# aws/sagemaker-xgboost-container

Hardware: NVIDIA H100
Metric: boosting rounds/sec (higher is better)
Workload: dtype int64

## Files before the change

### sagemaker-xgboost-container_b200/csrc/grow.cu

```cuda
#include "grow.h"
#include <algorithm>
#include <cmath>
#include <cstdlib>
#include <cstring>
#include "comm.h"

namespace b200 {

__global__ void pack_tree_kernel(TreeArrays t, const int* n_nodes, DevNode* out, int cap) {
  const int nn = *n_nodes;
  for (int i = blockIdx.x * blockDim.x + threadIdx.x; i < cap; i += gridDim.x * blockDim.x) {
    DevNode d;
    if (i < nn) { d.cond = t.split_cond[i]; d.left = t.left[i]; d.right = t.right[i]; d.fidx_dl = (unsigned)t.split_index[i] | ((unsigned)t.default_left[i] << 31); }
    else { d.cond = 0.f; d.left = -1; d.right = -1; d.fidx_dl = 0; }
    out[i] = d;
  }
}
__global__ void snapshot_h_kernel(const GH64* slot, long long* cache, size_t entries) {
  for (size_t e = (size_t)blockIdx.x * blockDim.x + threadIdx.x; e < entries; e += (size_t)gridDim.x * blockDim.x) cache[e] = slot[e].h;
}
__global__ void slot_from_cache_kernel(GH64* slot, const long long* cache, size_t entries) {
  for (size_t e = (size_t)blockIdx.x * blockDim.x + threadIdx.x; e < entries; e += (size_t)gridDim.x * blockDim.x) { GH64 v; v.g = 0; v.h = cache[e]; slot[e] = v; }
}
__global__ void gather_u32_kernel(const unsigned* src, const unsigned* idx, unsigned* dst, int64_t n) {
  const int64_t i = (int64_t)blockIdx.x * blockDim.x + threadIdx.x;
  if (i < n) dst[i] = src[idx[i]];
}

void* PinnedPool::take(size_t bytes) {
  bytes = (bytes + 255) & ~(size_t)255;
  while (cur < chunks.size() && off + bytes > chunks[cur].second) { ++cur; off = 0; }
  if (cur >= chunks.size()) { size_t sz = std::max<size_t>(bytes, 4u << 20); char* p = nullptr; CUDA_OK(cudaMallocHost(&p, sz)); chunks.emplace_back(p, sz); off = 0; }
  void* r = chunks[cur].first + off; off += bytes; return r;
}
static bool tail_by_position(const BinnedMatrix& bm) { return bm.tw == 4 && !bm.tail_in_gather; }

size_t TreeBuilder::carve(GrowState& gs, uintptr_t base) const {
  const size_t N = cap_nodes, L = max_level_nodes, nblocks = ngroups + (tw > 0 ? 1 : 0);
  size_t off = 0;
  auto take = [&](auto*& p, size_t bytes) { p = reinterpret_cast<std::remove_reference_t<decltype(p)>>(base + off); off += (bytes + 255) & ~(size_t)255; };
  take(gs.seg_begin, 4 * N); take(gs.seg_count, 4 * N); take(gs.hist_slot, 4 * N); take(gs.node_sum, 16 * N); take(gs.root_gain, 4 * N); take(gs.weight, 4 * N);
  take(gs.best, sizeof(SplitCand) * N); take(gs.best_group, sizeof(SplitCand) * N * nblocks);
  take(gs.level_nodes, 4 * (size_t)(kMaxDepth + 1) * L); take(gs.level_count, 4 * (kMaxDepth + 2));
  take(gs.build_nid, 4 * L); take(gs.build_sub_nid, 4 * L); take(gs.build_parent_slot, 4 * L); take(gs.build_count, 4); take(gs.build_prefix, 4 * (L + 1));
  take(gs.part_action, 4 * L); take(gs.tile_prefix, 4 * (L + 1));
  take(gs.tile_desc, 8 * ((size_t)max_tiles + 1)); gs.part_ctl = (unsigned*)(gs.tile_desc + max_tiles);
  take(gs.n_leaves, 4); take(gs.scales, 16); take(gs.absmax, 8);
  take(gs.depth, 4 * N); take(gs.open, N); take(gs.n_slots, 4); take(gs.lg_done, 4); take(gs.lower, 4 * N); take(gs.upper, 4 * N);
  return off;
}

void TreeBuilder::ensure(const BinnedMatrix& bm, int max_depth_, int K, int lg_iters_, int n_ic_) {
  const bool tail_pos_ = tail_by_position(bm);
  const int64_t stride_ = (bm.n + 63) & ~(int64_t)63;
  if (n == bm.n && F == bm.F && ngroups == bm.ngroups && tw == bm.tw && tail_pos == tail_pos_ && max_depth == max_depth_ && lg_iters == lg_iters_ &&
      n_ic == n_ic_ && gpair.n >= (size_t)stride_ * K + 512) return;
  if (lg_iters_ == 0) B200_CHECK(max_depth_ >= 1 && max_depth_ <= kMaxDepth, "max_depth must be in [1, 16] for the B200 depth-wise hist builder");
  n = bm.n; F = bm.F; ngroups = bm.ngroups; tw = bm.tw; tail_pos = tail_pos_; max_depth = max_depth_; lg_iters = lg_iters_; n_ic = n_ic_;
  gp_stride = stride_; root_h_valid = false;
  cudaStream_t s = engine_stream();
  if (peer_reduce_active()) {
    peer_reduce_close();
    DevBuf<unsigned> bar; bar.alloc(1); bar.zero(s);
    Comm::get().allreduce_max_u32(bar.p, 1, s);
    Comm::get().sync_stream(s);
  }
  for (auto& tg : graphs) tg.destroy();
  size_t pool_slots; int max_nodes;
  if (lg_iters > 0) {
    max_nodes = 2 * lg_iters + 1; max_level_nodes = 2; region = 0;
    pool_slots = (size_t)lg_iters + kLgFirstFreeSlot;
  } else {
    max_nodes = (1 << (max_depth + 1)) - 1; max_level_nodes = 1 << (max_depth - 1); region = max_level_nodes;
    pool_slots = 2 * (size_t)region;
  }
  cap_nodes = (max_nodes + 15) & ~15;
  slot_stride = hist_slot_entries(ngroups, tw);
  const size_t pool_bytes = pool_slots * slot_stride * sizeof(GH64);
  size_t free_b = 0, total_b = 0; cudaMemGetInfo(&free_b, &total_b);
  B200_CHECK(pool_bytes < free_b / 2 + hist_pool.n * sizeof(GH64), "histogram pool for this max_depth / max_leaves / feature count does not fit in device memory");
  hist_pool.alloc(pool_slots * slot_stride);
  gpair.alloc((size_t)gp_stride * K + 512); gpair.zero(s); err.alloc(1); tree_index_dev.alloc(1);
  if (!leaf_scale.p) { leaf_scale.alloc(1); set_leaf_scale(1.0f); }
  root_h_cache.alloc(slot_stride);
  const bool routed = routes(lg_iters, max_depth);
  for (int i = 0; i < 2; ++i) { const size_t m = i == 0 || !routed ? (size_t)n : 0; ridx[i].alloc(m); gp[i].alloc(m); tl[i].alloc(tail_pos ? m : 0); }
  route_tiles = routed ? (unsigned)((n + kRouteTile - 1) / kRouteTile) : 0u;
  node_of_row.alloc(routed ? (size_t)n : 0);
  route_counts.alloc(routed && max_depth >= 2 ? ((size_t)1 << (max_depth - 2)) * route_tiles : 0);
  max_tiles = (unsigned)((n + kPartTile - 1) / kPartTile) + max_level_nodes + 1;
  scratch.alloc(3 * (size_t)max_level_nodes + 8);
  state_block.alloc(carve(gs, 0)); state_block.zero(s);
  carve(gs, (uintptr_t)state_block.p);
  tree_block.alloc(tree_block_bytes(cap_nodes));
  const TreeBlock tb = tree_block_layout(tree_block.p, cap_nodes);
  gs.n_nodes = tb.n_nodes; ta = tb.t; packed.alloc(cap_nodes);
  ic_path.alloc(n_ic ? (size_t)cap_nodes * F : 0); ic_allowed.alloc(n_ic ? (size_t)cap_nodes * F : 0);
  ic_sets.alloc((size_t)n_ic * F); ic_sets_host.clear();
  hist_configure();
  global_n = n;
  if (Comm::get().distributed()) {
    peer_reduce_setup({{hist_pool.p, hist_pool.n * sizeof(GH64)}, {state_block.p, state_block.n}}, s);
    DevBuf<double> dsum; dsum.alloc(1); double v = (double)n;
    CUDA_OK(cudaMemcpyAsync(dsum.p, &v, sizeof v, cudaMemcpyHostToDevice, s));
    Comm::get().allreduce_sum_f64(dsum.p, 1, s);
    CUDA_OK(cudaMemcpyAsync(&v, dsum.p, sizeof v, cudaMemcpyDeviceToHost, s));
    Comm::get().sync_stream(s);
    global_n = (int64_t)v;
  }
}

float* TreeBuilder::ensure_adaptive() {
  if (adapt.ensure(n, max_leaves(), cap_nodes)) for (auto& tg : graphs) tg.destroy();
  return adapt.resid.p;
}

void TreeBuilder::set_leaf_scale(float v) {
  cudaStream_t s = engine_stream();
  CUDA_OK(cudaMemcpyAsync(leaf_scale.p, &v, sizeof v, cudaMemcpyHostToDevice, s));
  Comm::get().sync_stream(s);
}

const unsigned char* TreeBuilder::upload_mask(const std::string& mask, int tree_index) {
  cudaStream_t s = engine_stream(); feat_mask.ensure(mask.size());
  CUDA_OK(cudaMemcpyAsync(feat_mask.p, mask.data(), mask.size(), cudaMemcpyHostToDevice, s));
  CUDA_OK(cudaMemcpyAsync(tree_index_dev.p, &tree_index, sizeof(int), cudaMemcpyHostToDevice, s));
  Comm::get().sync_stream(s); return feat_mask.p;
}
template <typename T> static T* upload_changed(DevBuf<T>& d, std::vector<T>& host, const std::vector<T>& v) {
  if (v == host && d.n >= v.size()) return d.p;
  cudaStream_t s = engine_stream(); d.ensure(v.size());
  CUDA_OK(cudaMemcpyAsync(d.p, v.data(), sizeof(T) * v.size(), cudaMemcpyHostToDevice, s));
  Comm::get().sync_stream(s); host = v; return d.p;
}

const int* TreeBuilder::upload_monotone(const std::vector<int>& mono, int F_) {
  if (mono.empty()) return nullptr;
  B200_CHECK((int)mono.size() <= F_, "monotone_constraints has more entries than the data has features");
  std::vector<int> mh(mono); mh.resize((size_t)F_, 0);
  return upload_changed(monotone_dev, monotone_host, mh);
}
void TreeBuilder::upload_interaction(const std::vector<std::vector<int>>& ic, int F_) {
  if (ic.empty()) return;
  std::vector<unsigned char> sets(ic.size() * (size_t)F_, 0);
  for (size_t si = 0; si < ic.size(); ++si)
    for (int f : ic[si]) { B200_CHECK(f < F_, "interaction_constraints names feature " + std::to_string(f) + " but the data has " + std::to_string(F_) + " features"); sets[si * F_ + f] = 1; }
  upload_changed(ic_sets, ic_sets_host, sets);
}
HistArgs TreeBuilder::hist_args(const BinnedMatrix& bm, int k) const {
  HistArgs ha{}; ha.bins = bm.bins; ha.bins_tail = bm.bins_tail; ha.n = bm.n; ha.row_stride = bm.ngroups * kSlots; ha.tw = bm.tw;
  ha.bins_gather = bm.bins_gather; ha.gather_stride = bm.gather_stride;
  ha.tail_in_gather = bm.tail_in_gather;
  ha.gpair = gpair.p + (size_t)k * gp_stride;
  ha.build_count = gs.build_count; ha.build_nid = gs.build_nid; ha.build_prefix = gs.build_prefix; ha.seg_begin = gs.seg_begin;
  ha.hist_slot = gs.hist_slot; ha.scales = gs.scales; ha.hist_pool = hist_pool.p; ha.node_sum = gs.node_sum; ha.ngroups = bm.ngroups;
  ha.accumulate_sum = 1; ha.window_rows = window_rows_for(global_n);
  return ha;
}

EvalArgs TreeBuilder::eval_args(const TreeInputs& in, int level, const unsigned char* feat_mask) const {
  const BinnedMatrix& bm = in.bm;
  EvalArgs ea{}; ea.hist_pool = hist_pool.p; ea.gs = gs; ea.cut_ptrs = in.cut_ptrs; ea.feat_mask = feat_mask; ea.p = in.p; ea.F = bm.F;
  ea.ngroups = bm.ngroups; ea.tw = bm.tw; ea.ntail = bm.ntail; ea.has_missing = bm.has_missing; ea.level = level; ea.max_level_nodes = max_level_nodes;
  ea.colsample_bynode = in.mask ? in.colsample_bynode : 1.0f; ea.seed = in.seed; ea.tree_index = tree_index_dev.p; ea.monotone = in.monotone;
  ea.node_allowed = in.n_ic > 0 ? ic_allowed.p : nullptr;
  return ea;
}
ApplyArgs TreeBuilder::apply_args(const TreeInputs& in, int level, int next_base, int next_half) const {
  const BinnedMatrix& bm = in.bm;
  ApplyArgs aa{}; aa.gs = gs; aa.tree = ta; aa.cut_ptrs = in.cut_ptrs; aa.cut_vals = in.cut_vals; aa.min_vals = in.min_vals;
  aa.p = in.p; aa.scratch = scratch.p; aa.nblocks = bm.ngroups + (bm.tw > 0 ? 1 : 0); aa.level = level; aa.max_level_nodes = max_level_nodes;
  aa.next_base = next_base; aa.next_half = next_half; aa.monotone = in.monotone;
  if (in.n_ic > 0) { aa.node_path = ic_path.p; aa.node_allowed = ic_allowed.p; aa.ic_sets = ic_sets.p; aa.n_ic_sets = in.n_ic; aa.F = bm.F; }
  return aa;
}
template <class Launch> void TreeBuilder::timed(ProfKind kind, Launch launch) {
  if (!profile) { launch(); return; }
  ProfEvent e; e.kind = kind; e.launches = g_kernel_launches;
  CUDA_OK(cudaEventCreate(&e.a)); CUDA_OK(cudaEventCreate(&e.b));
  CUDA_OK(cudaEventRecord(e.a, engine_stream()));
  launch();
  e.launches = g_kernel_launches - e.launches;
  CUDA_OK(cudaEventRecord(e.b, engine_stream()));
  prof_events.push_back(e);
}

constexpr int kRootRows = -1;
void TreeBuilder::enqueue(const TreeInputs& in) {
  cudaStream_t s = engine_stream();
  const BinnedMatrix& bm = in.bm;
  const int k = in.k, D = in.p.max_depth;
  const bool dist = in.world > 1;
  const int num_sms = engine_num_sms();
  launch_init_tree(gs, ta, (unsigned)bm.n, s);
  if (in.root_mode == 2) { slot_from_cache_kernel<<<num_sms, 256, 0, s>>>(hist_pool.p, root_h_cache.p, slot_stride); ++g_kernel_launches; CUDA_OK(cudaGetLastError()); }
  else CUDA_OK(cudaMemsetAsync(hist_pool.p, 0, slot_stride * sizeof(GH64), s));
  const bool g_only = in.root_mode != 0;
  const int pay = g_only ? 4 : 8;
  const bool carry_tail = tail_by_position(bm);
  const bool routed = routes(in.lg_iters, D);
  if (profile && routed) {
    prof_part_row_bytes[0] = 3;
    prof_part_row_bytes[1] = 4;
    prof_part_row_bytes[2] = pay + 4 + pay + (carry_tail ? 8 : 0);
  } else if (profile) {
    prof_part_row_bytes[0] = pay + (carry_tail ? 4 : 0) + 1;
    prof_part_row_bytes[2] = 4 + pay + (carry_tail ? 4 : 0);
    prof_part_row_bytes[1] = prof_part_row_bytes[2] + 1;
  }
  HistArgs root = hist_args(bm, k);
  if (g_only) { root.gpair = nullptr; root.gpos = g_dense(); }
  root.g_only = in.root_mode == 2 ? 1 : 0; root.rows_counter = profile ? prof_rows.p : nullptr;
  timed(kProfRootHist, [&] { launch_hist_build(root, num_sms, s); });
  if (in.root_mode == 1) { snapshot_h_kernel<<<num_sms, 256, 0, s>>>(hist_pool.p, root_h_cache.p, slot_stride); ++g_kernel_launches; CUDA_OK(cudaGetLastError()); }
  auto collective = [&](std::function<void()> f) {
    if (!dist) return;
    if (!capturing) { f(); return; }
    end_segment(); capturing->colls.push_back(f);
    CUDA_OK(cudaStreamBeginCapture(s, cudaStreamCaptureModeThreadLocal));
  };
  auto allreduce_hist = [&](GH64* p, size_t cnt) {
    if (!dist) return;
    if (peer_allreduce_i64(reinterpret_cast<long long*>(p), cnt, s)) return;
    collective([p, cnt, s]() { Comm::get().allreduce_sum_i64(p, cnt, s); });
  };
  allreduce_hist(hist_pool.p, slot_stride * 2);
  allreduce_hist(gs.node_sum, 2);
  if (in.n_ic > 0) {
    CUDA_OK(cudaMemsetAsync(ic_path.p, 0, (size_t)bm.F, s));
    CUDA_OK(cudaMemsetAsync(ic_allowed.p, 1, (size_t)bm.F, s));
  }
  auto part_args = [&](int level, int cur, int next) {
    const bool root = cur == kRootRows;
    PartArgs pa{}; pa.gs = gs; pa.tree = ta; pa.bins_col = bm.bins_col; pa.n = bm.n;
    pa.ridx_cur = root ? nullptr : ridx[cur].p; pa.ridx_next = ridx[next].p;
    const void* root_gp = g_only ? static_cast<const void*>(g_dense()) : static_cast<const void*>(gpair.p + (size_t)k * gp_stride);
    pa.gp_cur = root ? root_gp : gp[cur].p; pa.gp_next = gp[next].p; pa.g_only = g_only ? 1 : 0;
    pa.tl_cur = !carry_tail ? nullptr : (root ? reinterpret_cast<const unsigned*>(bm.bins_tail) : tl[cur].p); pa.tl_next = carry_tail ? tl[next].p : nullptr;
    pa.has_missing = bm.has_missing; pa.level = level; pa.max_level_nodes = max_level_nodes; pa.rows_counter = profile ? prof_rows.p + 2 : nullptr;
    return pa;
  };
  auto level_hist_args = [&](int set) {
    HistArgs ha = hist_args(bm, k);
    ha.ridx = ridx[set].p; ha.tail_pos = carry_tail ? tl[set].p : nullptr; ha.accumulate_sum = 0;
    ha.gpair = g_only ? nullptr : gp[set].p; ha.gpos = g_only ? reinterpret_cast<const float*>(gp[set].p) : nullptr;
    ha.rows_counter = profile ? prof_rows.p + 1 : nullptr;
    return ha;
  };
  launch_eval(eval_args(in, 0, in.mask), 1, s);
  for (int it = 0; it < in.lg_iters; ++it) {
    launch_apply_lossguide(apply_args(in, 0, 0, 0), it, s);
    const PartArgs pa = part_args(0, it == 0 ? kRootRows : 0, 1);
    timed(kProfPartition, [&] { launch_partition(pa, max_tiles, s); });
    launch_lg_copy_back(pa, ridx[0].p, gp[0].p, tl[0].p, max_tiles, s);
    launch_zero_build_slots(gs, hist_pool.p, slot_stride, 1, s);
    timed(kProfDeepHist, [&] { launch_hist_build(level_hist_args(0), num_sms, s); });
    if (dist) {
      launch_lg_stage(gs, hist_pool.p, slot_stride, 1, s);
      allreduce_hist(hist_pool.p + (size_t)kLgStageSlot * slot_stride, slot_stride * 2);
      launch_lg_stage(gs, hist_pool.p, slot_stride, 0, s);
    }
    launch_subtract(gs, hist_pool.p, slot_stride, 1, s);
    launch_eval(eval_args(in, 1, nullptr), 2, s);
  }
  for (int L = 0; L < D && in.lg_iters == 0; ++L) {
    const bool final_level = (L == D - 1);
    const int next_base = ((L + 1) & 1) * region, next_half = 1 << L;
    launch_apply(apply_args(in, L, next_base, next_half), s);
    if (final_level) break;
    if (routed) {
      RouteArgs ra{}; ra.gs = gs; ra.tree = ta; ra.bins_col = bm.bins_col; ra.n = bm.n; ra.node_of_row = node_of_row.p;
      ra.tile_counts = route_counts.p; ra.ntiles = route_tiles; ra.has_missing = bm.has_missing; ra.level = L;
      if (g_only) ra.g = g_dense(); else ra.gpair = gpair.p + (size_t)k * gp_stride;
      ra.g_only = g_only ? 1 : 0;
      ra.tail_row = carry_tail ? reinterpret_cast<const unsigned*>(bm.bins_tail) : nullptr;
      ra.ridx = ridx[0].p; ra.gp = gp[0].p; ra.tl = carry_tail ? tl[0].p : nullptr; ra.rows_counter = profile ? prof_rows.p + 2 : nullptr;
      timed(kProfPartition, [&] { launch_route(ra, s); });
    } else {
      PartArgs pa = part_args(L, L == 0 ? kRootRows : (L & 1) ^ 1, L & 1);
      pa.build_only = L == D - 2 ? 1 : 0;
      timed(kProfPartition, [&] { launch_partition(pa, max_tiles, s); });
    }
    CUDA_OK(cudaMemsetAsync(hist_pool.p + (size_t)next_base * slot_stride, 0, (size_t)next_half * slot_stride * sizeof(GH64), s));
    timed(kProfDeepHist, [&] { launch_hist_build(level_hist_args(routed ? 0 : L & 1), num_sms, s); });
    allreduce_hist(hist_pool.p + (size_t)next_base * slot_stride, (size_t)next_half * slot_stride * 2);
    launch_subtract(gs, hist_pool.p, slot_stride, next_half, s);
    launch_eval(eval_args(in, L + 1, in.mask ? in.mask + (size_t)(L + 1) * bm.F : nullptr), 1 << (L + 1), s);
  }
  const uint8_t* start = routed && D >= 2 ? node_of_row.p : nullptr;
  if (in.adaptive) {
    launch_locate_leaves(ta, gs.n_nodes, bm.bins_col, bm.n, bm.has_missing, start, g_only ? nullptr : gpair.p + (size_t)k * gp_stride, &adapt, s);
    SelectArgs sa{}; sa.values = in.resid; sa.seg = adapt.seg.p; sa.h = in.adaptive == 2 ? reinterpret_cast<const float*>(gpair.p + (size_t)k * gp_stride) + 1 : nullptr;
    sa.h_stride = 2; sa.scales = gs.scales; sa.n = bm.n; sa.nseg = max_leaves(); sa.alpha = 0.5;
    if (in.adaptive == 3) { sa.h = in.weight; sa.h_stride = 1; sa.scales = adapt.scales.p; }
    sa.leaf_nid = adapt.leaf_nid.p; sa.split_cond = ta.split_cond; sa.lr = in.p.eta;
    segmented_select(sa, &adapt, [&](unsigned long long* p, size_t cnt) { collective([p, cnt, s]() { Comm::get().allreduce_sum_i64(p, cnt, s); }); },
                     [&](unsigned* p, size_t cnt) { collective([p, cnt, s]() { Comm::get().allreduce_max_u32(p, cnt, s); }); }, s);
  }
  timed(kProfMargin, [&] { launch_update_margin(ta, gs.n_nodes, bm.bins_col, bm.n, bm.has_missing, start, in.margin, in.K, k, leaf_scale.p, s); });
  if (profile) prof_margin_rows += bm.n;
  pack_tree_kernel<<<(cap_nodes + 255) / 256, 256, 0, s>>>(ta, gs.n_nodes, packed.p, cap_nodes); ++g_kernel_launches;
  CUDA_OK(cudaGetLastError());
}
void TreeBuilder::end_segment() {
  cudaGraph_t graph = nullptr; cudaGraphExec_t exec = nullptr;
  CUDA_OK(cudaStreamEndCapture(engine_stream(), &graph));
  cudaError_t e = cudaGraphInstantiate(&exec, graph, 0);
  cudaGraphDestroy(graph);
  CUDA_OK(e);
  capturing->segs.push_back(exec);
}

void TreeBuilder::grow(const TreeInputs& in) {
  cudaStream_t s = engine_stream();
  static const bool no_graph = getenv("B200XGB_NO_GRAPH") != nullptr;
  if ((int)graphs.size() <= in.k) graphs.resize(in.k + 1);
  TreeGraph& tg = graphs[in.k];
  if (profile || no_graph || (in.world > 1 && !tg.eager_done) || in.root_mode == 1) { tg.eager_done = true; enqueue(in); return; }
  if (tg.segs.empty() || memcmp(&tg.key, &in, sizeof in) != 0) {
    tg.destroy();
    const long long launches_before = g_kernel_launches;
    CUDA_OK(cudaStreamBeginCapture(s, cudaStreamCaptureModeThreadLocal));
    capturing = &tg;
    try { enqueue(in); end_segment(); }
    catch (...) { capturing = nullptr; cudaGraph_t graph = nullptr; cudaStreamEndCapture(s, &graph); if (graph) cudaGraphDestroy(graph); tg.destroy(); throw; }
    capturing = nullptr;
    tg.key = in; tg.launches = g_kernel_launches - launches_before;
    g_kernel_launches = launches_before;
  }
  for (size_t i = 0; i < tg.segs.size(); ++i) {
    CUDA_OK(cudaGraphLaunch(tg.segs[i], s));
    if (i < tg.colls.size()) tg.colls[i]();
  }
  g_kernel_launches += tg.launches;
}
PendingTree TreeBuilder::stage_tree() {
  cudaStream_t s = engine_stream();
  PendingTree pt; pt.cap_nodes = (size_t)cap_nodes; pt.staging = pinned.take(tree_block.n);
  if (!free_events.empty()) { pt.ready = free_events.back(); free_events.pop_back(); }
  else CUDA_OK(cudaEventCreateWithFlags(&pt.ready, cudaEventDisableTiming));
  CUDA_OK(cudaMemcpyAsync(pt.staging, tree_block.p, tree_block.n, cudaMemcpyDeviceToHost, s));
  CUDA_OK(cudaEventRecord(pt.ready, s));
  return pt;
}

void TreeBuilder::debug_build_root_hist(const BinnedMatrix& bm, const float* gpair_host, std::vector<long long>* hist_out, float* scales_out,
                                        int repeats, float* ms_out, int mode, const unsigned* row_ids, int64_t n_ids) {
  cudaStream_t s = engine_stream();
  const int64_t rows = row_ids ? n_ids : bm.n;
  B200_CHECK(rows <= bm.n, "debug_build_root_hist: more row ids than rows");
  CUDA_OK(cudaMemcpyAsync(gpair.p, gpair_host, sizeof(float2) * rows, cudaMemcpyHostToDevice, s));
  if (row_ids) CUDA_OK(cudaMemcpyAsync(ridx[0].p, row_ids, sizeof(unsigned) * rows, cudaMemcpyHostToDevice, s));
  float mg = 0.f, mh = 0.f;
  for (int64_t i = 0; i < rows; ++i) { mg = std::max(mg, std::fabs(gpair_host[2 * i])); mh = std::max(mh, gpair_host[2 * i + 1]); }
  unsigned am[2]; memcpy(&am[0], &mg, 4); memcpy(&am[1], &mh, 4);
  CUDA_OK(cudaMemcpyAsync(gs.absmax, am, 8, cudaMemcpyHostToDevice, s));
  launch_scales(gs, grad_bits_for(global_n), s);
  HistArgs ha = hist_args(bm, 0);
  ha.ridx = row_ids ? ridx[0].p : nullptr;
  ha.force_gather = (mode & 3) == 1 ? 1 : 0; ha.g_only = (mode & 3) == 2 ? 1 : 0;
  if ((mode & 8) || ha.g_only) {
    std::vector<float> gh((size_t)rows);
    for (int64_t i = 0; i < rows; ++i) gh[i] = gpair_host[2 * i];
    float* gpos = row_ids ? reinterpret_cast<float*>(gp[0].p) : g_dense();
    if (rows) CUDA_OK(cudaMemcpyAsync(gpos, gh.data(), sizeof(float) * rows, cudaMemcpyHostToDevice, s));
    Comm::get().sync_stream(s);
    ha.gpos = gpos; ha.gpair = nullptr;
  }
  if ((mode & 4) && row_ids && tail_by_position(bm)) {
    gather_u32_kernel<<<(unsigned)((rows + 255) / 256), 256, 0, s>>>(reinterpret_cast<const unsigned*>(bm.bins_tail), ridx[0].p, tl[0].p, rows); ++g_kernel_launches;
    CUDA_OK(cudaGetLastError());
    ha.tail_pos = tl[0].p;
  }
  root_h_valid = false;
  cudaEvent_t e0, e1; CUDA_OK(cudaEventCreate(&e0)); CUDA_OK(cudaEventCreate(&e1));
  float total = 0.f;
  for (int r = 0; r < std::max(1, repeats); ++r) {
    launch_init_tree(gs, ta, (unsigned)rows, s);
    CUDA_OK(cudaMemsetAsync(hist_pool.p, 0, slot_stride * sizeof(GH64), s));
    CUDA_OK(cudaEventRecord(e0, s));
    launch_hist_build(ha, engine_num_sms(), s);
    CUDA_OK(cudaEventRecord(e1, s));
    CUDA_OK(cudaEventSynchronize(e1));
    float ms = 0; CUDA_OK(cudaEventElapsedTime(&ms, e0, e1)); total += ms;
  }
  if (ms_out) *ms_out = total / std::max(1, repeats);
  hist_out->resize(slot_stride * 2);
  CUDA_OK(cudaMemcpyAsync(hist_out->data(), hist_pool.p, sizeof(GH64) * slot_stride, cudaMemcpyDeviceToHost, s));
  CUDA_OK(cudaMemcpyAsync(scales_out, gs.scales, 4 * sizeof(float), cudaMemcpyDeviceToHost, s));
  Comm::get().sync_stream(s);
  cudaEventDestroy(e0); cudaEventDestroy(e1);
}

std::string TreeBuilder::debug_eval_root(const TreeInputs& in, const long long* hist_fm, long long G, long long H, float max_g, float max_h,
                                         float lower, float upper) {
  cudaStream_t s = engine_stream();
  root_h_valid = false;
  const BinnedMatrix& bm = in.bm;
  const int F_ = bm.F;
  std::vector<GH64> slot(slot_stride, GH64{0, 0});
  const size_t W = (size_t)bm.ngroups * kSlots, tail0 = (size_t)bm.ngroups * kGroupEntries;
  for (int f = 0; f < F_; ++f)
    for (int b = 0; b < kBins; ++b) {
      const size_t e = (size_t)f < W ? ((size_t)(f / kSlots) * kBins + b) * kSlots + f % kSlots : tail0 + (size_t)b * bm.tw + (f - W);
      slot[e].g = hist_fm[((size_t)f * kBins + b) * 2]; slot[e].h = hist_fm[((size_t)f * kBins + b) * 2 + 1];
    }
  launch_init_tree(gs, ta, (unsigned)bm.n, s);
  CUDA_OK(cudaMemcpyAsync(hist_pool.p, slot.data(), sizeof(GH64) * slot_stride, cudaMemcpyHostToDevice, s));
  const GH64 tot{G, H};
  CUDA_OK(cudaMemcpyAsync(gs.node_sum, &tot, sizeof tot, cudaMemcpyHostToDevice, s));
  CUDA_OK(cudaMemcpyAsync(gs.lower, &lower, 4, cudaMemcpyHostToDevice, s));
  CUDA_OK(cudaMemcpyAsync(gs.upper, &upper, 4, cudaMemcpyHostToDevice, s));
  unsigned am[2]; memcpy(&am[0], &max_g, 4); memcpy(&am[1], &max_h, 4);
  CUDA_OK(cudaMemcpyAsync(gs.absmax, am, 8, cudaMemcpyHostToDevice, s));
  launch_scales(gs, grad_bits_for(global_n), s);
  launch_eval(eval_args(in, 0, in.mask), 1, s);
  const ApplyArgs aa = apply_args(in, 0, region, 1);
  if (in.lg_iters > 0) launch_apply_lossguide(aa, 0, s); else launch_apply(aa, s);
  const int nblocks = bm.ngroups + (bm.tw > 0 ? 1 : 0);
  std::vector<unsigned char> sb(state_block.n), tb(tree_block.n);
  CUDA_OK(cudaMemcpyAsync(sb.data(), state_block.p, sb.size(), cudaMemcpyDeviceToHost, s));
  CUDA_OK(cudaMemcpyAsync(tb.data(), tree_block.p, tb.size(), cudaMemcpyDeviceToHost, s));
  Comm::get().sync_stream(s);
  GrowState h; carve(h, (uintptr_t)sb.data());
  auto bits = [](float v) { unsigned u; memcpy(&u, &v, 4); return std::to_string(u); };
  auto cand = [&](const SplitCand& c) {
    return "{\"loss_chg\":" + bits(c.loss_chg) + ",\"feature\":" + std::to_string(c.feature) + ",\"bin\":" + std::to_string(c.bin) + ",\"dleft\":" +
           std::to_string(c.dleft) + ",\"ord\":" + std::to_string(c.ord) + ",\"GL\":" + std::to_string(c.GL) + ",\"HL\":" + std::to_string(c.HL) + "}";
  };
  const TreeBlock t = tree_block_layout(tb.data(), cap_nodes);
  const int nn = *t.n_nodes;
  std::string o = "{\"scales\":[";
  for (int i = 0; i < 4; ++i) o += (i ? "," : "") + bits(h.scales[i]);
  o += "],\"root_gain\":" + bits(h.root_gain[0]) + ",\"weight\":" + bits(h.weight[0]) + ",\"best_group\":[";
  for (int i = 0; i < nblocks; ++i) o += (i ? "," : "") + cand(h.best_group[i]);
  o += "],\"best\":" + cand(h.best[0]) + ",\"n_nodes\":" + std::to_string(nn) + ",\"expanded\":" + (nn == 3 ? "true" : "false") + ",\"tree\":{";
  const char* iname[5] = {"left", "right", "parent", "split_index", "split_bin"};
  const int* iarr[5] = {t.t.left, t.t.right, t.t.parent, t.t.split_index, t.t.split_bin};
  const char* fname[4] = {"split_cond", "base_weight", "loss_chg", "sum_hess"};
  const float* farr[4] = {t.t.split_cond, t.t.base_weight, t.t.loss_chg, t.t.sum_hess};
  for (int a = 0; a < 5; ++a) { o += std::string(a ? "," : "") + "\"" + iname[a] + "\":["; for (int i = 0; i < nn; ++i) o += (i ? "," : "") + std::to_string(iarr[a][i]); o += "]"; }
  for (int a = 0; a < 4; ++a) { o += std::string(",\"") + fname[a] + "\":["; for (int i = 0; i < nn; ++i) o += (i ? "," : "") + bits(farr[a][i]); o += "]"; }
  o += ",\"default_left\":["; for (int i = 0; i < nn; ++i) o += (i ? "," : "") + std::to_string((int)t.t.default_left[i]); o += "]}";
  o += ",\"children\":[";
  for (int c = 1; c < nn && c < 3; ++c)
    o += std::string(c > 1 ? "," : "") + "{\"G\":" + std::to_string(h.node_sum[c].g) + ",\"H\":" + std::to_string(h.node_sum[c].h) + ",\"lower\":" + bits(h.lower[c]) + ",\"upper\":" + bits(h.upper[c]) + "}";
  o += "]}";
  return o;
}

void TreeBuilder::set_profile(bool on) {
  profile = on;
  if (on) { prof_rows.alloc(4); prof_rows.zero(engine_stream()); prof_margin_rows = 0; }
  for (auto& e : prof_events) { cudaEventDestroy(e.a); cudaEventDestroy(e.b); }
  prof_events.clear();
}
std::string TreeBuilder::profile_json() {
  cudaStream_t s = engine_stream();
  Comm::get().sync_stream(s);
  double ms[kProfKinds] = {}; long long launches[kProfKinds] = {};
  for (auto& e : prof_events) { float t = 0; CUDA_OK(cudaEventElapsedTime(&t, e.a, e.b)); ms[e.kind] += t; launches[e.kind] += e.launches; }
  unsigned long long rows[4] = {0, 0, 0, 0};
  if (prof_rows.p) CUDA_OK(cudaMemcpy(rows, prof_rows.p, sizeof rows, cudaMemcpyDeviceToHost));
  char buf[1024];
  snprintf(buf, sizeof buf, "{\"root_hist_ms\":%.6f,\"root_hist_launches\":%lld,\"root_hist_rows\":%llu,\"deep_hist_ms\":%.6f,\"deep_hist_launches\":%lld,\"deep_hist_rows\":%llu,"
           "\"part_ms\":%.6f,\"part_launches\":%lld,\"part_rows\":%llu,\"part_rows_written\":%llu,"
           "\"part_row_bytes_in_root\":%d,\"part_row_bytes_in\":%d,\"part_row_bytes_out\":%d,\"margin_ms\":%.6f,\"margin_launches\":%lld,\"margin_rows\":%lld}",
           ms[kProfRootHist], launches[kProfRootHist], rows[0], ms[kProfDeepHist], launches[kProfDeepHist], rows[1],
           ms[kProfPartition], launches[kProfPartition], rows[2], rows[3], prof_part_row_bytes[0], prof_part_row_bytes[1], prof_part_row_bytes[2],
           ms[kProfMargin], launches[kProfMargin], prof_margin_rows);
  return buf;
}

}
```

### sagemaker-xgboost-container_b200/csrc/grow.h

```cpp
#pragma once
#include <functional>
#include <string>
#include <type_traits>
#include <vector>
#include "adaptive.h"
#include "engine.h"
#include "misc.h"
#include "tree.h"

namespace b200 {

struct TreeInputs {
  BinnedMatrix bm;
  const int* cut_ptrs; const float* cut_vals; const float* min_vals;
  float* margin;
  const unsigned char* mask;
  const int* monotone;
  TrainParamDev p;
  float colsample_bynode; unsigned seed;
  int lg_iters, n_ic;
  int K, k, world;
  int root_mode;
  const float* resid; const float* weight;
  int adaptive;
  int unused;
};
static_assert(std::is_trivially_copyable<TreeInputs>::value, "TreeInputs is compared as bytes");
static_assert(sizeof(BinnedMatrix) == 4 * sizeof(void*) + sizeof(int64_t) + 8 * sizeof(int), "BinnedMatrix has padding bytes");
static_assert(sizeof(TrainParamDev) == 8 * 4, "TrainParamDev has padding bytes");
static_assert(sizeof(TreeInputs) == sizeof(BinnedMatrix) + 8 * sizeof(void*) + sizeof(TrainParamDev) + 10 * 4, "TreeInputs has padding bytes");

inline size_t tree_block_bytes(size_t cap) { return 64 + 9 * 4 * cap + cap; }
struct TreeBlock { int* n_nodes; TreeArrays t; };
inline TreeBlock tree_block_layout(void* base, size_t cap) {
  int* ip = (int*)((unsigned char*)base + 64); float* fp = (float*)(ip + 5 * cap);
  return {(int*)base, {ip, ip + cap, ip + 2 * cap, ip + 3 * cap, ip + 4 * cap, (unsigned char*)(fp + 4 * cap), fp, fp + cap, fp + 2 * cap, fp + 3 * cap}};
}

struct PendingTree {
  void* staging = nullptr; size_t cap_nodes = 0; cudaEvent_t ready = nullptr;
};
struct PinnedPool {
  std::vector<std::pair<char*, size_t>> chunks; size_t cur = 0, off = 0;
  ~PinnedPool() { for (auto& c : chunks) cudaFreeHost(c.first); }
  void* take(size_t bytes);
  void reset() { cur = 0; off = 0; }
};

struct TreeGraph {
  std::vector<cudaGraphExec_t> segs; std::vector<std::function<void()>> colls;
  TreeInputs key{}; long long launches = 0;
  bool eager_done = false;
  TreeGraph() = default; TreeGraph(TreeGraph&&) = default;
  ~TreeGraph() { destroy(); }
  void destroy() { for (auto e : segs) if (e) cudaGraphExecDestroy(e); segs.clear(); colls.clear(); }
};

struct TreeBuilder {
  int64_t n = 0; int F = 0, ngroups = 0, tw = 0, max_depth = 0, cap_nodes = 0, max_level_nodes = 0, region = 0; bool tail_pos = false;
  int lg_iters = 0, n_ic = 0;
  size_t slot_stride = 0;
  int64_t gp_stride = 0;
  unsigned max_tiles = 0;
  int64_t global_n = 0;
  DevBuf<long long> root_h_cache; uint64_t root_h_uid = 0, root_h_version = 0; bool root_h_valid = false;
  GrowState gs{}; TreeArrays ta{};
  DevBuf<unsigned char> state_block;
  DevBuf<unsigned char> tree_block;
  DevBuf<GH64> hist_pool; DevBuf<unsigned> ridx[2], scratch;
  DevBuf<float2> gpair, gp[2]; DevBuf<unsigned> tl[2]; DevBuf<int> err, tree_index_dev; DevBuf<unsigned char> ic_path, ic_allowed, ic_sets;
  DevBuf<uint8_t> node_of_row; DevBuf<unsigned> route_counts; unsigned route_tiles = 0;
  DevBuf<DevNode> packed;
  DevBuf<float> leaf_scale;
  DevBuf<unsigned char> feat_mask; DevBuf<int> monotone_dev;
  std::vector<unsigned char> ic_sets_host;
  std::vector<int> monotone_host;
  PinnedPool pinned; std::vector<cudaEvent_t> free_events;
  std::vector<TreeGraph> graphs;
  TreeGraph* capturing = nullptr;
  SelectScratch adapt;
  int max_leaves() const { return lg_iters > 0 ? lg_iters + 1 : 1 << max_depth; }
  float* ensure_adaptive();
  enum ProfKind { kProfRootHist, kProfDeepHist, kProfPartition, kProfMargin, kProfKinds };
  struct ProfEvent { cudaEvent_t a, b; int kind; long long launches; };
  bool profile = false; std::vector<ProfEvent> prof_events;
  DevBuf<unsigned long long> prof_rows;
  long long prof_margin_rows = 0;
  int prof_part_row_bytes[3] = {0, 0, 0};

  ~TreeBuilder() { for (auto e : free_events) cudaEventDestroy(e); for (auto& e : prof_events) { cudaEventDestroy(e.a); cudaEventDestroy(e.b); } }
  void ensure(const BinnedMatrix& bm, int max_depth, int K, int lg_iters, int n_ic);
  static bool routes(int lg_iters, int max_depth) { return lg_iters == 0 && max_depth <= kRouteMaxDepth; }
  const unsigned char* upload_mask(const std::string& mask, int tree_index);
  const int* upload_monotone(const std::vector<int>& mono, int F);
  void upload_interaction(const std::vector<std::vector<int>>& sets, int F);
  void set_leaf_scale(float v);
  void grow(const TreeInputs& in);
  PendingTree stage_tree();
  void set_profile(bool on); std::string profile_json();
  void debug_build_root_hist(const BinnedMatrix& bm, const float* gpair_host, std::vector<long long>* hist_out, float* scales_out,
                             int repeats, float* ms_out, int mode, const unsigned* row_ids, int64_t n_ids);
  std::string debug_eval_root(const TreeInputs& in, const long long* hist_fm, long long G, long long H, float max_g, float max_h,
                              float lower, float upper);

 private:
  size_t carve(GrowState& g, uintptr_t base) const;
  void enqueue(const TreeInputs& in);
  void end_segment();
  HistArgs hist_args(const BinnedMatrix& bm, int k) const;
  float* g_dense() const { return reinterpret_cast<float*>(gpair.p); }
  EvalArgs eval_args(const TreeInputs& in, int level, const unsigned char* feat_mask) const;
  ApplyArgs apply_args(const TreeInputs& in, int level, int next_base, int next_half) const;
  template <class Launch> void timed(ProfKind kind, Launch launch);
};

}
```

### sagemaker-xgboost-container_b200/csrc/hist.cu

```cuda
#include <cuda.h>
#include <cstdlib>
#include <cstring>
#include <map>
#include <mutex>
#include <tuple>
#include <type_traits>
#include "engine.h"
#include "tree.h"

namespace b200 {

constexpr int kSuperRows = 32;
constexpr int kMinRowsPerCta = 4096;
constexpr int kSpillThreshold = 1 << 24;
constexpr int kPlaneBytes = kGroupEntries * 4;
constexpr int kMaxSmem = 232448;
constexpr int kTeamWarps = 4, kTeams = 6, kRootRows = 16 * kTeamWarps;
constexpr int kRootConsumerWarps = kTeamWarps * kTeams;
constexpr int kRootProducerWarps = 3;
constexpr int kRootThreads = (kRootConsumerWarps + kRootProducerWarps) * 32;

template <int K, int N, typename F> __device__ __forceinline__ void static_for(F&& f) {
  if constexpr (K < N) { f(std::integral_constant<int, K>{}); static_for<K + 1, N>(f); }
}

__device__ __forceinline__ uint4 ldg_nc_v4(const void* p) {
  uint4 r;
  asm volatile("ld.global.nc.L1::no_allocate.v4.u32 {%0,%1,%2,%3}, [%4];" : "=r"(r.x), "=r"(r.y), "=r"(r.z), "=r"(r.w) : "l"(p));
  return r;
}
__device__ __forceinline__ uint2 ldg_nc_v2(const void* p) {
  uint2 r;
  asm volatile("ld.global.nc.L1::no_allocate.v2.u32 {%0,%1}, [%2];" : "=r"(r.x), "=r"(r.y) : "l"(p));
  return r;
}
__device__ __forceinline__ unsigned ldg_nc_u32(const void* p) {
  unsigned r;
  asm volatile("ld.global.nc.L1::no_allocate.u32 %0, [%1];" : "=r"(r) : "l"(p));
  return r;
}
__device__ __forceinline__ float2 ldg_nc_f2(const void* p) {
  float2 r;
  asm volatile("ld.global.nc.L1::no_allocate.v2.f32 {%0,%1}, [%2];" : "=f"(r.x), "=f"(r.y) : "l"(p));
  return r;
}
__device__ __forceinline__ uint4 lds_v4(unsigned addr) {
  uint4 r;
  asm volatile("ld.shared.v4.u32 {%0,%1,%2,%3}, [%4];" : "=r"(r.x), "=r"(r.y), "=r"(r.z), "=r"(r.w) : "r"(addr));
  return r;
}
__device__ __forceinline__ uint2 lds_v2(unsigned addr) {
  uint2 r;
  asm volatile("ld.shared.v2.u32 {%0,%1}, [%2];" : "=r"(r.x), "=r"(r.y) : "r"(addr));
  return r;
}
__device__ __forceinline__ unsigned lds_u32(unsigned addr) {
  unsigned r;
  asm volatile("ld.shared.u32 %0, [%1];" : "=r"(r) : "r"(addr));
  return r;
}
__device__ __forceinline__ void red_shared_s32(unsigned addr, int v) {
  asm volatile("red.shared.add.s32 [%0], %1;" :: "r"(addr), "r"(v) : "memory");
}
template <int OFF> __device__ __forceinline__ void red_shared_s32_off(unsigned addr, int v) {
  asm volatile("red.shared.add.s32 [%0+%2], %1;" :: "r"(addr), "r"(v), "n"(OFF) : "memory");
}
template <int OFF> __device__ __forceinline__ void red_shared_u32_off(unsigned addr, unsigned v) {
  asm volatile("red.shared.add.u32 [%0+%2], %1;" :: "r"(addr), "r"(v), "n"(OFF) : "memory");
}
__device__ __forceinline__ void red_shared_u32(unsigned addr, unsigned v) {
  asm volatile("red.shared.add.u32 [%0], %1;" :: "r"(addr), "r"(v) : "memory");
}
__device__ __forceinline__ void red_global_s64(long long* p, long long v) {
  asm volatile("red.global.add.u64 [%0], %1;" :: "l"(p), "l"(v) : "memory");
}
__device__ __forceinline__ void mbar_init(unsigned bar, unsigned count) {
  asm volatile("mbarrier.init.shared::cta.b64 [%0], %1;" :: "r"(bar), "r"(count) : "memory");
}
__device__ __forceinline__ void mbar_expect_tx(unsigned bar, unsigned bytes) {
  asm volatile("mbarrier.arrive.expect_tx.shared::cta.b64 _, [%0], %1;" :: "r"(bar), "r"(bytes) : "memory");
}
__device__ __forceinline__ void mbar_arrive(unsigned bar) {
  asm volatile("mbarrier.arrive.shared::cta.b64 _, [%0];" :: "r"(bar) : "memory");
}
__device__ __forceinline__ void mbar_wait(unsigned bar, unsigned parity) {
  asm volatile(
      "{\n"
      ".reg .pred P1;\n"
      "LAB_WAIT:\n"
      "mbarrier.try_wait.parity.shared::cta.b64 P1, [%0], %1;\n"
      "@P1 bra DONE;\n"
      "bra LAB_WAIT;\n"
      "DONE:\n"
      "}\n" :: "r"(bar), "r"(parity) : "memory");
}
__device__ __forceinline__ void tma_load_2d(unsigned dst, const CUtensorMap* tm, int c0, int c1, unsigned bar) {
  asm volatile("cp.async.bulk.tensor.2d.shared::cluster.global.tile.mbarrier::complete_tx::bytes [%0], [%1, {%2, %3}], [%4];"
               :: "r"(dst), "l"(tm), "r"(c0), "r"(c1), "r"(bar) : "memory");
}
__device__ __forceinline__ void tma_prefetch_2d(const CUtensorMap* tm, int c0, int c1) {
  asm volatile("cp.async.bulk.prefetch.tensor.2d.L2.global.tile [%0, {%1, %2}];" :: "l"(tm), "r"(c0), "r"(c1) : "memory");
}
__device__ __forceinline__ void bulk_load_1d(unsigned dst, const void* src, unsigned bytes, unsigned bar) {
  asm volatile("cp.async.bulk.shared::cluster.global.mbarrier::complete_tx::bytes [%0], [%1], %2, [%3];"
               :: "r"(dst), "l"(src), "r"(bytes), "r"(bar) : "memory");
}
__device__ __forceinline__ void named_bar_sync(int id, int nthreads) {
  asm volatile("bar.sync %0, %1;" :: "r"(id), "r"(nthreads) : "memory");
}

struct LaneConst { unsigned A[16]; unsigned S[4]; int qw; };

__device__ __forceinline__ LaneConst make_lane_const_rot(int rot, int half, unsigned smem_base) {
  LaneConst lc;
  lc.qw = rot >> 2;
  const int qb = rot & 3;
#pragma unroll
  for (int jb = 0; jb < 4; ++jb) lc.S[jb] = 0x4440u | (unsigned)((jb + qb) & 3);
#pragma unroll
  for (int jw = 0; jw < 4; ++jw)
#pragma unroll
    for (int jb = 0; jb < 4; ++jb)
      lc.A[4 * jw + jb] = smem_base + 64u * (unsigned)half + 16u * (unsigned)((jw + lc.qw) & 3) + 4u * (unsigned)((jb + qb) & 3);
#pragma unroll
  for (int i = 0; i < 16; ++i) asm volatile("" : "+r"(lc.A[i]));
#pragma unroll
  for (int i = 0; i < 4; ++i) asm volatile("" : "+r"(lc.S[i]));
  return lc;
}
__device__ __forceinline__ LaneConst make_lane_const(int lane, unsigned smem_base) { return make_lane_const_rot(lane >> 1, lane & 1, smem_base); }

__device__ __forceinline__ void rotate_words(const LaneConst& lc, const uint4& w, unsigned (&ww)[4]) {
  unsigned w0 = w.x, w1 = w.y, w2 = w.z, w3 = w.w;
  if (lc.qw & 1) { unsigned x = w0; w0 = w1; w1 = w2; w2 = w3; w3 = x; }
  if (lc.qw & 2) { unsigned x = w0; w0 = w2; w2 = x; x = w1; w1 = w3; w3 = x; }
  ww[0] = w0; ww[1] = w1; ww[2] = w2; ww[3] = w3;
}

__device__ __forceinline__ void rotate_words_bytes(int qw, int qb8, const uint4& w, unsigned (&ww)[4]) {
  unsigned w0 = w.x, w1 = w.y, w2 = w.z, w3 = w.w;
  if (qw & 1) { unsigned x = w0; w0 = w1; w1 = w2; w2 = w3; w3 = x; }
  if (qw & 2) { unsigned x = w0; w0 = w2; w2 = x; x = w1; w1 = w3; w3 = x; }
  ww[0] = __funnelshift_r(w0, w0, qb8); ww[1] = __funnelshift_r(w1, w1, qb8); ww[2] = __funnelshift_r(w2, w2, qb8); ww[3] = __funnelshift_r(w3, w3, qb8);
}
template <int GOFF>
__device__ __forceinline__ void accumulate16_pairs_prerotated(const unsigned (&A)[16], const unsigned (&ww)[4], int gq, unsigned hq) {
#pragma unroll
  for (int jw = 0; jw < 4; ++jw) {
#pragma unroll
    for (int jb = 0; jb < 4; ++jb) {
      const unsigned bin = (ww[jw] >> (8 * jb)) & 0xffu;
      const unsigned addr = (bin << 7) + A[4 * jw + jb];
      red_shared_s32_off<GOFF>(addr, gq);
      red_shared_u32_off<GOFF + 32768>(addr, hq);
    }
  }
}

template <bool GONLY, int GOFF>
__device__ __forceinline__ void accumulate16(const LaneConst& lc, const unsigned (&ww)[4], int gq, unsigned hq) {
#pragma unroll
  for (int jw = 0; jw < 4; ++jw) {
#pragma unroll
    for (int jb = 0; jb < 4; ++jb) {
      const unsigned bin = __byte_perm(ww[jw], 0u, lc.S[jb]);
      const unsigned addr = (bin << 7) + lc.A[4 * jw + jb];
      red_shared_s32_off<GOFF>(addr, gq);
      if (!GONLY) red_shared_u32_off<GOFF + 32768>(addr, hq);
    }
  }
}

struct TailConst { unsigned base_g, hplane_bytes, bin_stride, rep_off; int tw; };

template <bool GONLY>
__device__ __forceinline__ void tail_accumulate(const TailConst& tc, int lane, unsigned w0, unsigned w1, int gq, unsigned hq) {
#pragma unroll
  for (int j = 0; j < 8; ++j) {
    if (j < tc.tw) {
      const unsigned slot = (unsigned)(j + lane) & (unsigned)(tc.tw - 1);
      const unsigned bin = __byte_perm(w0, w1, slot) & 0xffu;
      const unsigned addr = tc.base_g + bin * tc.bin_stride + tc.rep_off + slot * 4u;
      red_shared_s32(addr, gq);
      if (!GONLY) red_shared_u32(addr + tc.hplane_bytes, hq);
    }
  }
}

template <int TW, int TREP>
__device__ __forceinline__ void tail_accumulate_ct(unsigned base_rep, int lane, unsigned w0, unsigned w1, int gq, unsigned hq) {
  constexpr unsigned kBinStride = (unsigned)(TW * TREP) * 4u, kHPlane = 256u * kBinStride;
#pragma unroll
  for (int j = 0; j < TW; ++j) {
    const unsigned slot = (unsigned)(j + lane) & (unsigned)(TW - 1);
    const unsigned bin = __byte_perm(w0, w1, slot) & 0xffu;
    const unsigned addr = base_rep + bin * kBinStride + slot * 4u;
    red_shared_s32(addr, gq);
    red_shared_u32(addr + kHPlane, hq);
  }
}

__device__ __forceinline__ void flush_node_sum(GH64* dst, int g, unsigned h, int lane) {
  long long G = g, H = h;
#pragma unroll
  for (int o = 16; o > 0; o >>= 1) { G += __shfl_xor_sync(0xffffffffu, G, o); H += __shfl_xor_sync(0xffffffffu, H, o); }
  if (lane == 0 && (G != 0 || H != 0)) { red_global_s64(&dst->g, G); red_global_s64(&dst->h, H); }
}

template <int PL>
__device__ __forceinline__ void spill_main(int* smem, int ng_here, GH64* out, bool last, int tid, int nthr) {
  const int vecs = ng_here * PL * (kGroupEntries / 4);
  const int start = (int)(((long long)blockIdx.x * vecs) / gridDim.x);
  for (int i = tid; i < vecs; i += nthr) {
    int v = i + start; if (v >= vecs) v -= vecs;
    int4 x = reinterpret_cast<int4*>(smem)[v];
    if ((x.x | x.y | x.z | x.w) == 0) continue;
    const int plane = v >> 11;
    const int e0 = (v & 2047) << 2;
    const bool is_h = PL == 2 && (plane & 1);
    GH64* o = out + (size_t)(plane / PL) * kGroupEntries + e0;
    int vals[4] = {x.x, x.y, x.z, x.w};
    bool any = false;
#pragma unroll
    for (int k = 0; k < 4; ++k) {
      const int val = vals[k];
      const bool sp = last ? (val != 0) : (is_h ? ((unsigned)val >= (unsigned)kSpillThreshold) : (val >= kSpillThreshold || val <= -kSpillThreshold));
      if (sp) {
        red_global_s64(is_h ? &o[k].h : &o[k].g, is_h ? (long long)(unsigned)val : (long long)val);
        vals[k] = 0; any = true;
      }
    }
    if (any) reinterpret_cast<int4*>(smem)[v] = make_int4(vals[0], vals[1], vals[2], vals[3]);
  }
}

template <int PL>
__device__ __forceinline__ void spill_tail(int* tsm, int tw, int trep, GH64* out_tail, bool last, int tid, int nthr) {
  const int per_plane = 256 * tw * trep;
  const int per_bin = tw * trep;
  for (int idx = tid; idx < PL * per_plane; idx += nthr) {
    const int val = tsm[idx];
    if (val == 0) continue;
    const bool is_h = idx >= per_plane;
    const int e = is_h ? idx - per_plane : idx;
    const int bin = e / per_bin, slot = e & (tw - 1);
    const bool sp = last ? true : (is_h ? ((unsigned)val >= (unsigned)kSpillThreshold) : (val >= kSpillThreshold || val <= -kSpillThreshold));
    if (sp) {
      GH64* o = out_tail + bin * tw + slot;
      red_global_s64(is_h ? &o->h : &o->g, is_h ? (long long)(unsigned)val : (long long)val);
      tsm[idx] = 0;
    }
  }
}

struct RootCfg {
  int S;
  int trep;
  int box_groups;
  unsigned tail_off;
  unsigned ring_off;
  unsigned stage_bytes;
  unsigned total;
  int flags;
};

template <bool GONLY, int G>
__device__ __forceinline__ void root_unit(const LaneConst& lc, const unsigned (&ldsoff)[4], unsigned rowaddr, int gq, unsigned hq) {
  constexpr int PL = GONLY ? 1 : 2;
  unsigned ww[4];
#pragma unroll
  for (int j = 0; j < 4; ++j) ww[j] = lds_u32(rowaddr + (unsigned)(G * 32) + ldsoff[j]);
  accumulate16<GONLY, G * PL * kPlaneBytes>(lc, ww, gq, hq);
}

template <bool GONLY>
__global__ void __launch_bounds__(kRootThreads, 1)
hist_root_kernel(const __grid_constant__ CUtensorMap tm, HistArgs a, RootCfg c) {
  constexpr int PL = GONLY ? 1 : 2;
  constexpr int NCW = kRootConsumerWarps, R = kRootRows;
  extern __shared__ __align__(128) unsigned char smem_raw[];
  const int nb = *a.build_count;
  if (nb <= 0) return;
  const unsigned T = a.build_prefix[nb];
  if (T == 0) return;
  const int lane = threadIdx.x & 31, warp = threadIdx.x >> 5;
  const int g0 = blockIdx.y * a.ng_chunk;
  const int ng_here = min(a.ng_chunk, a.ngroups - g0);
  const bool has_tail = a.tw > 0 && blockIdx.y == gridDim.y - 1;
  if (a.rows_counter && blockIdx.x == 0 && blockIdx.y == 0 && threadIdx.x == 0) atomicAdd(a.rows_counter, (unsigned long long)T);

  const unsigned smem_base = (unsigned)__cvta_generic_to_shared(smem_raw);
  const unsigned ring = (smem_base + c.ring_off + 127u) & ~127u;
  const unsigned bars = ring + (unsigned)c.S * c.stage_bytes;
  const unsigned row_bytes = 32u * (unsigned)c.box_groups;
  const unsigned main_tile_bytes = (unsigned)R * row_bytes;
  constexpr unsigned kGradBytes = GONLY ? 4u : 8u;
  const unsigned gp_off = main_tile_bytes, tail_tile_off = main_tile_bytes + (unsigned)R * kGradBytes;
  const unsigned ntiles = (T + R - 1) / R;
  const unsigned my_ntiles = ntiles > blockIdx.x ? (ntiles - blockIdx.x + gridDim.x - 1) / gridDim.x : 0u;

  {
    const int main4 = ng_here * PL * kPlaneBytes / 16;
    int4* z = reinterpret_cast<int4*>(smem_raw);
    for (int i = threadIdx.x; i < main4; i += blockDim.x) z[i] = make_int4(0, 0, 0, 0);
    if (has_tail) {
      const int tail4 = PL * 256 * a.tw * c.trep * 4 / 16;
      int4* zt = reinterpret_cast<int4*>(smem_raw + c.tail_off);
      for (int i = threadIdx.x; i < tail4; i += blockDim.x) zt[i] = make_int4(0, 0, 0, 0);
    }
    if (threadIdx.x == 0) {
      for (int s = 0; s < c.S; ++s) { mbar_init(bars + 8u * s, 1); mbar_init(bars + 8u * (c.S + s), kTeamWarps); }
      asm volatile("fence.mbarrier_init.release.cluster;" ::: "memory");
    }
  }
  __syncthreads();

  const int nid = a.build_nid[0];
  const size_t slot_entries = (size_t)a.ngroups * kGroupEntries + (size_t)256 * a.tw;
  GH64* out_slot = a.hist_pool + (size_t)a.hist_slot[nid] * slot_entries;
  GH64* out_main = out_slot + (size_t)g0 * kGroupEntries;
  GH64* out_tail = out_slot + (size_t)a.ngroups * kGroupEntries;

  if (warp >= NCW) {
    if (lane == 0) {
      const unsigned P = (c.flags & 8) ? 1u : (unsigned)kRootProducerWarps, pw = (unsigned)(warp - NCW);
      if (pw < P) {
        const unsigned tx = main_tile_bytes + (unsigned)R * kGradBytes + (has_tail ? (unsigned)R * (unsigned)a.tw : 0u);
        unsigned s = pw % (unsigned)c.S, round = pw / (unsigned)c.S;
        for (unsigned i = pw; i < my_ntiles; i += P) {
          if (round > 0) mbar_wait(bars + 8u * (c.S + s), (round - 1u) & 1u);
          const unsigned full = bars + 8u * s, dst = ring + s * c.stage_bytes;
          const unsigned t = blockIdx.x + i * gridDim.x;
          const unsigned row0 = t * (unsigned)R;
          mbar_expect_tx(full, tx);
          if ((c.flags & 1) && gridDim.y == 1) bulk_load_1d(dst, a.bins + (size_t)row0 * a.row_stride, main_tile_bytes, full);
          else tma_load_2d(dst, &tm, g0 * 32, (int)row0, full);
          if (GONLY) bulk_load_1d(dst + gp_off, a.gpos + row0, (unsigned)R * 4u, full);
          else bulk_load_1d(dst + gp_off, a.gpair + row0, (unsigned)R * 8u, full);
          if (has_tail) bulk_load_1d(dst + tail_tile_off, a.bins_tail + (size_t)row0 * a.tw, (unsigned)R * (unsigned)a.tw, full);
          const unsigned tp = t + 8u * gridDim.x;
          if (tp < ntiles && !(c.flags & 4)) tma_prefetch_2d(&tm, g0 * 32, (int)(tp * (unsigned)R));
          s += P; if (s >= (unsigned)c.S) { s -= (unsigned)c.S; ++round; }
        }
      }
    }
    return;
  }

  const int team = warp / kTeamWarps, wit = warp % kTeamWarps;
  const float sg = a.scales[0], sh = a.scales[1];
  const LaneConst lc = make_lane_const(lane, smem_base);
  unsigned ldsoff[4];
#pragma unroll
  for (int j = 0; j < 4; ++j) { ldsoff[j] = 16u * (unsigned)(lane & 1) + 4u * (unsigned)((j + lc.qw) & 3); asm volatile("" : "+r"(ldsoff[j])); }
  TailConst tc;
  tc.tw = a.tw; tc.base_g = smem_base + c.tail_off; tc.hplane_bytes = 256u * (unsigned)a.tw * (unsigned)c.trep * 4u;
  tc.bin_stride = (unsigned)a.tw * (unsigned)c.trep * 4u;
  tc.rep_off = has_tail ? (unsigned)((lane / a.tw) % c.trep) * (unsigned)a.tw * 4u : 0u;
  const unsigned rowl = (unsigned)(wit << 4) + (unsigned)(lane >> 1);
  const unsigned tiles_per_window = (unsigned)a.window_rows / R;
  const unsigned hq_one = (unsigned)__float2int_rn(1.0f * sh);
  auto quant = [&](unsigned tile, unsigned row, bool valid, int& gq, unsigned& hq) {
    gq = 0; hq = 0;
    if constexpr (GONLY) {
      const float g = __uint_as_float(lds_u32(tile + gp_off + row * 4u));
      if (valid) { gq = __float2int_rn(g * sg); hq = hq_one; }
    } else {
      const uint2 gh = lds_v2(tile + gp_off + row * 8u);
      if (valid) { gq = __float2int_rn(__uint_as_float(gh.x) * sg); hq = (unsigned)__float2int_rn(__uint_as_float(gh.y) * sh); }
    }
  };
  long long accG = 0, accH = 0;
  unsigned i = (unsigned)team, s = (unsigned)team, ph = 0;
  for (unsigned wstart = 0;; wstart += tiles_per_window) {
    const unsigned wend = wstart + tiles_per_window < my_ntiles ? wstart + tiles_per_window : my_ntiles;
    while (i < wend) {
      mbar_wait(bars + 8u * s, ph);
      const unsigned tile = ring + s * c.stage_bytes;
      const unsigned row0 = (blockIdx.x + i * gridDim.x) * (unsigned)R;
      if (!(c.flags & 2)) {
        int gq; unsigned hq;
        quant(tile, rowl, row0 + rowl < T, gq, hq);
        if ((lane & 1) == 0) { accG += gq; accH += hq; }
        const unsigned rowaddr = tile + rowl * row_bytes;
        root_unit<GONLY, 0>(lc, ldsoff, rowaddr, gq, hq);
        if (ng_here > 1) root_unit<GONLY, 1>(lc, ldsoff, rowaddr, gq, hq);
        if (ng_here > 2) root_unit<GONLY, 2>(lc, ldsoff, rowaddr, gq, hq);
        if (has_tail) {
          const unsigned tu = ((unsigned)wit + i) & (unsigned)(kTeamWarps - 1);
          if (tu < (unsigned)(R >> 5)) {
            const unsigned trow = (tu << 5) + (unsigned)lane;
            unsigned w0, w1 = 0;
            if (a.tw == 4) w0 = lds_u32(tile + tail_tile_off + trow * 4u);
            else { const uint2 ww = lds_v2(tile + tail_tile_off + trow * 8u); w0 = ww.x; w1 = ww.y; }
            int gqt; unsigned hqt;
            quant(tile, trow, row0 + trow < T, gqt, hqt);
            if (row0 + trow >= T) { w0 = 0; w1 = 0; }
            tail_accumulate<GONLY>(tc, lane, w0, w1, gqt, hqt);
          }
        }
      }
      __syncwarp();
      if (lane == 0) mbar_arrive(bars + 8u * (c.S + s));
      i += kTeams; s += kTeams;
      if (s >= (unsigned)c.S) { s -= (unsigned)c.S; ph ^= 1u; }
    }
    if (wend == my_ntiles) break;
    named_bar_sync(1, NCW * 32);
    spill_main<PL>(reinterpret_cast<int*>(smem_raw), ng_here, out_main, false, threadIdx.x, NCW * 32);
    if (has_tail) spill_tail<PL>(reinterpret_cast<int*>(smem_raw + c.tail_off), a.tw, c.trep, out_tail, false, threadIdx.x, NCW * 32);
    named_bar_sync(1, NCW * 32);
  }
  named_bar_sync(1, NCW * 32);
  spill_main<PL>(reinterpret_cast<int*>(smem_raw), ng_here, out_main, true, threadIdx.x, NCW * 32);
  if (has_tail) spill_tail<PL>(reinterpret_cast<int*>(smem_raw + c.tail_off), a.tw, c.trep, out_tail, true, threadIdx.x, NCW * 32);
  if (a.accumulate_sum && blockIdx.y == 0) {
#pragma unroll
    for (int o = 16; o > 0; o >>= 1) { accG += __shfl_xor_sync(0xffffffffu, accG, o); accH += __shfl_xor_sync(0xffffffffu, accH, o); }
    if (lane == 0 && (accG != 0 || accH != 0)) { red_global_s64(&a.node_sum[nid].g, accG); red_global_s64(&a.node_sum[nid].h, accH); }
  }
}

template <int TW, bool GPAY> struct Stage { unsigned id; typename std::conditional<GPAY, float, float2>::type gr; unsigned t0; };
template <bool GPAY> struct Stage<8, GPAY> { unsigned id; typename std::conditional<GPAY, float, float2>::type gr; unsigned t0, t1; };

__host__ __device__ constexpr int gather_tail_replicas(int ng) { return ng >= 3 ? 4 : 8; }
__host__ __device__ constexpr int gather_tail_bytes(int ng) { return ng >= 3 ? 32768 : 65536; }

template <int NG, int TW, int NTHREADS, bool GPAY>
__global__ void __launch_bounds__(NTHREADS, NG == 1 ? (TW ? 1 : 3) : 1) hist_gather_kernel(HistArgs a) {
  constexpr bool TAIL = TW != 0;
  constexpr int NWARPS = NTHREADS / 32;
  constexpr int LPR = 2 * NG, RPI = 32 / LPR, U = 2 * NG;
  constexpr int SUP = RPI * U;
  static_assert(kWindowRowsSmall / (SUP * NWARPS) >= 1, "window too small");
  const unsigned iters_per_window = (unsigned)a.window_rows / (SUP * NWARPS);
  extern __shared__ __align__(16) int smem[];
  const int nb = *a.build_count;
  if (nb <= 0) return;
  const unsigned T = a.build_prefix[nb];
  if (T == 0) return;
  if (a.rows_counter && blockIdx.x == 0 && blockIdx.y == 0 && threadIdx.x == 0) atomicAdd(a.rows_counter, (unsigned long long)T);
  const unsigned C = gridDim.x;
  unsigned ceff = (T + kMinRowsPerCta - 1) / kMinRowsPerCta;
  ceff = ceff < 1 ? 1 : (ceff > C ? C : ceff);
  if (blockIdx.x >= ceff) return;
  unsigned chunk = (T + ceff - 1) / ceff;
  chunk = (chunk + SUP - 1) / SUP * SUP;
  unsigned long long r0l = (unsigned long long)blockIdx.x * chunk;
  if (r0l >= T) return;
  unsigned r0 = (unsigned)r0l;
  unsigned r1 = (unsigned long long)r0 + chunk > T ? T : r0 + chunk;
  const int g0 = blockIdx.y * a.ng_chunk;
  const int ng_here = min(min(a.ng_chunk, NG), a.ngroups - g0);
  const bool has_tail = TAIL && a.tw > 0 && blockIdx.y == gridDim.y - 1;
  const float sg = a.scales[0], sh = a.scales[1];
  const unsigned smem_g = (unsigned)__cvta_generic_to_shared(smem);
  const bool aligned = a.ridx != nullptr && a.bins_gather != nullptr;
  constexpr bool kLineTail = NG == 3 && TW == 8;
  const bool tail_line = kLineTail && aligned && a.tail_in_gather;
  const int64_t row_stride = aligned ? (int64_t)a.gather_stride : (int64_t)a.row_stride;
  const int lane = threadIdx.x & 31, warp = threadIdx.x >> 5;
  const int q = lane / LPR, c = lane - q * LPR;
  const bool lane_on = q < RPI && (c >> 1) < ng_here;
  const int rot = q < RPI ? NG * q + (c >> 1) : 15;
  const LaneConst lc = make_lane_const_rot(rot, c & 1, smem_g + (unsigned)((q < RPI ? (c >> 1) : 0) * 2 * kPlaneBytes));
  const int rot_qw = rot >> 2, rot_qb8 = (rot & 3) * 8;
  const uint8_t* gbins = (aligned ? a.bins_gather : a.bins) + (int64_t)g0 * kSlots + c * 16;
  constexpr int TWC = TAIL ? TW : 4;
  constexpr int trep = gather_tail_replicas(NG) < gather_tail_bytes(NG) / (2 * 256 * 4 * TWC) ? gather_tail_replicas(NG) : gather_tail_bytes(NG) / (2 * 256 * 4 * TWC);
  const unsigned tail_base_rep = smem_g + (unsigned)(NG * 2 * kPlaneBytes) + (unsigned)((lane / TWC) % trep) * (unsigned)TWC * 4u;

  {
    const int words4 = (NG * 2 * kPlaneBytes + (TAIL ? 2 * 256 * TWC * trep * 4 : 0)) / 16;
    for (int i = threadIdx.x; i < words4; i += NTHREADS) reinterpret_cast<int4*>(smem)[i] = make_int4(0, 0, 0, 0);
  }
  __syncthreads();

  int b = 0;
  { int lo = 0, hi = nb; while (lo < hi) { int mid = (lo + hi) >> 1; if (a.build_prefix[mid + 1] > r0) hi = mid; else lo = mid + 1; } b = lo; }

  const size_t slot_entries = (size_t)a.ngroups * kGroupEntries + (size_t)256 * a.tw;
  typedef Stage<TW, GPAY> StageT;
  const unsigned hq_one = (unsigned)__float2int_rn(1.0f * sh);
  while (r0 < r1) {
    const unsigned nbeg = a.build_prefix[b], nend_node = a.build_prefix[b + 1];
    const unsigned nend = nend_node < r1 ? nend_node : r1;
    const int nid = a.build_nid[b];
    const unsigned seg = a.seg_begin[nid];
    GH64* out_slot = a.hist_pool + (size_t)a.hist_slot[nid] * slot_entries;
    GH64* out_main = out_slot + (size_t)g0 * kGroupEntries;
    GH64* out_tail = out_slot + (size_t)a.ngroups * kGroupEntries;
    int accG = 0; unsigned accH = 0;
    const unsigned pa = seg + (r0 - nbeg), pb = seg + (nend - nbeg);
    const unsigned nsuper = (pb - pa + SUP - 1) / SUP;
    const unsigned iters = (nsuper + NWARPS - 1) / NWARPS;

    auto load_ids = [&](unsigned st) -> StageT {
      StageT s_; s_.id = 0xffffffffu; s_.gr = {}; s_.t0 = 0u;
      if constexpr (TW == 8) s_.t1 = 0u;
      unsigned p = pa + st * SUP + lane;
      if (lane < SUP && st < nsuper && p < pb) {
        s_.id = a.ridx ? __ldg(a.ridx + p) : p;
        if constexpr (GPAY) s_.gr = __uint_as_float(ldg_nc_u32(a.gpos + p)); else s_.gr = ldg_nc_f2(a.gpair + p);
        if (TAIL && has_tail && !tail_line) {
          if constexpr (TW == 8) { const uint2 v = ldg_nc_v2(a.bins_tail + (int64_t)s_.id * 8); s_.t0 = v.x; s_.t1 = v.y; }
          else if (a.tail_pos) s_.t0 = ldg_nc_u32(a.tail_pos + p);
          else s_.t0 = ldg_nc_u32(a.bins_tail + (int64_t)s_.id * 4);
        }
      }
      return s_;
    };
    auto load_unit = [&](unsigned ids, int k) -> uint4 {
      const unsigned rid = __shfl_sync(0xffffffffu, ids, q < RPI ? k * RPI + q : 0);
      return (lane_on && rid != 0xffffffffu) ? ldg_nc_v4(gbins + (int64_t)rid * row_stride) : make_uint4(0, 0, 0, 0);
    };
    auto load_line_tail = [&](StageT& s_) {
      if constexpr (TAIL) {
        if (tail_line && has_tail && s_.id != 0xffffffffu) {
          const uint8_t* t = a.bins_gather + (int64_t)s_.id * row_stride + a.ngroups * kSlots;
          if constexpr (TW == 8) { const uint2 v = ldg_nc_v2(t); s_.t0 = v.x; s_.t1 = v.y; } else s_.t0 = ldg_nc_u32(t);
        }
      }
    };
    StageT cur = load_ids(warp);
    StageT nxt = load_ids(warp + NWARPS);
    uint4 w[U];
#pragma unroll
    for (int k = 0; k < U; ++k) w[k] = load_unit(cur.id, k);
    load_line_tail(cur);
    for (unsigned it = 0; it < iters; ++it) {
      const unsigned s = warp + it * NWARPS;
      StageT nn = load_ids(s + 2 * NWARPS);
      const bool active = s < nsuper;
      int gq_l; unsigned hq_l;
      if constexpr (GPAY) { gq_l = __float2int_rn(cur.gr * sg); hq_l = cur.id != 0xffffffffu ? hq_one : 0u; }
      else { gq_l = __float2int_rn(cur.gr.x * sg); hq_l = (unsigned)__float2int_rn(cur.gr.y * sh); }
      accG += gq_l; accH += hq_l;
#pragma unroll
      for (int k = 0; k < U; ++k) {
        if (active) {
          int gq = __shfl_sync(0xffffffffu, gq_l, q < RPI ? k * RPI + q : 0);
          unsigned hq = __shfl_sync(0xffffffffu, hq_l, q < RPI ? k * RPI + q : 0);
          if (!lane_on) { gq = 0; hq = 0; }
          unsigned ww[4];
          rotate_words_bytes(rot_qw, rot_qb8, w[k], ww);
          accumulate16_pairs_prerotated<0>(lc.A, ww, gq, hq);
        }
        w[k] = load_unit(nxt.id, k);
      }
      if constexpr (TAIL) { if (active && has_tail) { unsigned t1 = 0; if constexpr (TW == 8) t1 = cur.t1; tail_accumulate_ct<TWC, trep>(tail_base_rep, lane, cur.t0, t1, gq_l, hq_l); } }
      load_line_tail(nxt);
      cur = nxt; nxt = nn;
      if ((it + 1) % iters_per_window == 0 && it + 1 < iters) {
        if (a.accumulate_sum && blockIdx.y == 0) { flush_node_sum(a.node_sum + nid, accG, accH, lane); accG = 0; accH = 0; }
        __syncthreads();
        spill_main<2>(smem, ng_here, out_main, false, threadIdx.x, NTHREADS);
        if (has_tail) spill_tail<2>(smem + NG * 2 * kGroupEntries, TWC, trep, out_tail, false, threadIdx.x, NTHREADS);
        __syncthreads();
      }
    }
    __syncthreads();
    spill_main<2>(smem, ng_here, out_main, true, threadIdx.x, NTHREADS);
    if (has_tail) spill_tail<2>(smem + NG * 2 * kGroupEntries, TWC, trep, out_tail, true, threadIdx.x, NTHREADS);
    __syncthreads();
    if (a.accumulate_sum && blockIdx.y == 0) flush_node_sum(a.node_sum + nid, accG, accH, lane);
    r0 = nend; ++b;
  }
}

static thread_local const char* g_last_kernel = "none";
const char* hist_last_kernel() { return g_last_kernel; }

static int chunks_for(int ngroups) { return (ngroups + 2) / 3; }
static int groups_per_chunk(int ngroups) { const int nc = chunks_for(ngroups); return (ngroups + nc - 1) / nc; }

static bool root_plan(int ngc, int tw, bool gonly, RootCfg* c) {
  const int PL = gonly ? 1 : 2;
  const unsigned main_b = (unsigned)ngc * PL * kPlaneBytes;
  const unsigned avail = kMaxSmem - 128  - 2 * 8 * 16 ;
  const unsigned stage = (unsigned)kRootRows * (32u * ngc + (gonly ? 4u : 8u) + tw);
  int trep = tw ? 32 / tw : 0;
  unsigned tail_b = (unsigned)PL * 256u * tw * trep * 4u;
  if (tw && main_b + tail_b + kTeams * stage > avail) { trep = 1; tail_b = (unsigned)PL * 256u * tw * 4u; }
  if (main_b + tail_b + kTeams * stage > avail) return false;
  int S = (int)((avail - main_b - tail_b) / stage);
  int smax = 16;
  if (const char* e = getenv("B200XGB_ROOT_S")) smax = atoi(e);
  if (S > smax) S = smax;
  constexpr int kStageQuantum = kTeams % kRootProducerWarps == 0 ? kTeams : kTeams * kRootProducerWarps;
  S -= S % kStageQuantum;
  if (S < kTeams) return false;
  c->S = S; c->trep = trep; c->box_groups = ngc; c->tail_off = main_b; c->ring_off = main_b + tail_b; c->stage_bytes = stage;
  c->total = main_b + tail_b + 128 + (unsigned)S * stage + 2 * 8 * (unsigned)S;
  c->flags = 0;
  if (const char* f = getenv("B200XGB_ROOT_FLAGS")) c->flags = atoi(f);
  return true;
}

typedef CUresult (*EncodeTiledFn)(CUtensorMap*, CUtensorMapDataType, cuuint32_t, void*, const cuuint64_t*, const cuuint64_t*, const cuuint32_t*,
                                  const cuuint32_t*, CUtensorMapInterleave, CUtensorMapSwizzle, CUtensorMapL2promotion, CUtensorMapFloatOOBfill);
static EncodeTiledFn encode_fn() {
  static EncodeTiledFn fn = [] {
    void* p = nullptr; cudaDriverEntryPointQueryResult q;
    if (cudaGetDriverEntryPoint("cuTensorMapEncodeTiled", &p, cudaEnableDefault, &q) != cudaSuccess || q != cudaDriverEntryPointSuccess) { cudaGetLastError(); p = nullptr; }
    return reinterpret_cast<EncodeTiledFn>(p);
  }();
  return fn;
}

static bool get_tensor_map(const uint8_t* bins, int64_t n, int row_stride, int box_groups, int R, CUtensorMap* out) {
  typedef std::tuple<const void*, int64_t, int, int, int> Key;
  static std::map<Key, CUtensorMap> cache; static std::mutex mu;
  std::lock_guard<std::mutex> lk(mu);
  const Key key(bins, n, row_stride, box_groups, R);
  auto it = cache.find(key);
  if (it != cache.end()) { *out = it->second; return true; }
  EncodeTiledFn fn = encode_fn();
  if (!fn) return false;
  CUtensorMap tm;
  const cuuint64_t dims[2] = {(cuuint64_t)row_stride, (cuuint64_t)n};
  const cuuint64_t strides[1] = {(cuuint64_t)row_stride};
  const cuuint32_t box[2] = {(cuuint32_t)(32 * box_groups), (cuuint32_t)R};
  const cuuint32_t estr[2] = {1, 1};
  CUresult r = fn(&tm, CU_TENSOR_MAP_DATA_TYPE_UINT8, 2, const_cast<uint8_t*>(bins), dims, strides, box, estr, CU_TENSOR_MAP_INTERLEAVE_NONE,
                  CU_TENSOR_MAP_SWIZZLE_NONE, CU_TENSOR_MAP_L2_PROMOTION_L2_128B, CU_TENSOR_MAP_FLOAT_OOB_FILL_NONE);
  if (r != CUDA_SUCCESS) return false;
  if (cache.size() > 64) cache.clear();
  cache[key] = tm; *out = tm;
  return true;
}

template <int NG, int TW, int NT> static void set_gather_attr() {
  const int smem = NG * 2 * kPlaneBytes + (TW ? gather_tail_bytes(NG) : 0);
  CUDA_OK(cudaFuncSetAttribute(hist_gather_kernel<NG, TW, NT, false>, cudaFuncAttributeMaxDynamicSharedMemorySize, smem));
  CUDA_OK(cudaFuncSetAttribute(hist_gather_kernel<NG, TW, NT, true>, cudaFuncAttributeMaxDynamicSharedMemorySize, smem));
}

void hist_configure() {
  static bool configured = false;
  if (configured) return;
  set_gather_attr<1, 0, 256>(); set_gather_attr<1, 4, 256>(); set_gather_attr<1, 8, 256>();
  set_gather_attr<2, 0, 768>(); set_gather_attr<2, 4, 768>(); set_gather_attr<2, 8, 768>();
  set_gather_attr<3, 0, 768>(); set_gather_attr<3, 4, 768>(); set_gather_attr<3, 8, 768>();
  CUDA_OK(cudaFuncSetAttribute(hist_root_kernel<false>, cudaFuncAttributeMaxDynamicSharedMemorySize, kMaxSmem));
  CUDA_OK(cudaFuncSetAttribute(hist_root_kernel<true>, cudaFuncAttributeMaxDynamicSharedMemorySize, kMaxSmem));
  configured = true;
}

template <int NG, int NT, bool GPAY>
static void launch_gather_tw(const HistArgs& a, int gx, int nchunks, cudaStream_t stream) {
  const int smem = NG * 2 * kPlaneBytes + (a.tw ? gather_tail_bytes(NG) : 0);
  if (a.tw == 0) hist_gather_kernel<NG, 0, NT, GPAY><<<dim3(gx, nchunks), NT, smem, stream>>>(a);
  else if (a.tw == 4) hist_gather_kernel<NG, 4, NT, GPAY><<<dim3(gx, nchunks), NT, smem, stream>>>(a);
  else hist_gather_kernel<NG, 8, NT, GPAY><<<dim3(gx, nchunks), NT, smem, stream>>>(a);
}
template <int NG, int NT>
static void launch_gather(const HistArgs& a, int gx, int nchunks, cudaStream_t stream) {
  if (a.gpos) launch_gather_tw<NG, NT, true>(a, gx, nchunks, stream); else launch_gather_tw<NG, NT, false>(a, gx, nchunks, stream);
}

void launch_hist_build(const HistArgs& a_in, int num_sms, cudaStream_t stream) {
  HistArgs a = a_in;
  const int nchunks = chunks_for(a.ngroups);
  a.ng_chunk = groups_per_chunk(a.ngroups);
  static const bool no_tma = getenv("B200XGB_NO_TMA") != nullptr;
  const bool gonly = a.g_only != 0;
  B200_CHECK(!gonly || a.gpos != nullptr, "hist: the G-only root pass reads the dense g (gpos)");
  if (a.ridx == nullptr && !no_tma && !a.force_gather && (a.gpos == nullptr || gonly)) {
    RootCfg c; CUtensorMap tm;
    if (root_plan(a.ng_chunk, a.tw, gonly, &c) && get_tensor_map(a.bins, a.n, a.row_stride, c.box_groups, kRootRows, &tm)) {
      const int gx = num_sms / nchunks > 0 ? num_sms / nchunks : 1;
      if (gonly) hist_root_kernel<true><<<dim3(gx, nchunks), kRootThreads, c.total, stream>>>(tm, a, c);
      else hist_root_kernel<false><<<dim3(gx, nchunks), kRootThreads, c.total, stream>>>(tm, a, c);
      g_last_kernel = gonly ? "hist_root_kernel<GONLY>" : "hist_root_kernel<GH>";
      ++g_kernel_launches;
      CUDA_OK(cudaGetLastError());
      return;
    }
  }
  B200_CHECK(!a.g_only || a.ridx == nullptr, "hist: G-only accumulation is a root-pass mode");
  B200_CHECK(!a.g_only, "hist: the G-only root pass needs the TMA kernel (tensor-map creation failed or B200XGB_NO_TMA is set)");
  const bool tail = a.tw > 0;
  const int ng = a.ng_chunk;
  if (ng == 1) {
    const int per_sm = tail ? 1 : 3;
    const int gx = (num_sms * per_sm + nchunks - 1) / nchunks;
    launch_gather<1, 256>(a, gx, nchunks, stream);
  } else {
    const int gx = (num_sms + nchunks - 1) / nchunks;
    if (ng == 2) launch_gather<2, 768>(a, gx, nchunks, stream); else launch_gather<3, 768>(a, gx, nchunks, stream);
  }
  g_last_kernel = "hist_gather_kernel";
  ++g_kernel_launches;
  CUDA_OK(cudaGetLastError());
}

}
```

### sagemaker-xgboost-container_b200/csrc/tree.h

```cpp
#pragma once
#include "engine.h"

namespace b200 {

constexpr unsigned kPartTile = 2048;

struct TrainParamDev {
  float eta, lambda, alpha, gamma, min_child_weight, max_delta_step;
  int max_depth, max_leaves;
};

struct EvalArgs {
  const GH64* hist_pool; GrowState gs; const int* cut_ptrs; const unsigned char* feat_mask;
  TrainParamDev p; int F, ngroups, tw, ntail, has_missing, level, max_level_nodes;
  const int* monotone;
  const unsigned char* node_allowed;
  float colsample_bynode; unsigned seed; const int* tree_index;
};

struct ApplyArgs {
  GrowState gs; TreeArrays tree; const int* cut_ptrs; const float* cut_vals; const float* min_vals;
  TrainParamDev p; unsigned* scratch; int nblocks , level, max_level_nodes, next_base, next_half;
  const int* monotone;
  unsigned char* node_path; unsigned char* node_allowed; const unsigned char* ic_sets; int n_ic_sets, F;
};

struct PartArgs {
  GrowState gs; TreeArrays tree; const uint8_t* bins_col; int64_t n; const unsigned* ridx_cur; unsigned* ridx_next;
  const void* gp_cur; void* gp_next; int g_only;
  const unsigned* tl_cur; unsigned* tl_next;
  int has_missing, level, max_level_nodes;
  int build_only;
  unsigned long long* rows_counter;
};

constexpr int kRouteMaxDepth = 7;
constexpr unsigned kRouteTile = 2048;
constexpr int kRouteMaxNodes = 256;
constexpr int kRouteMaxBuild = 1 << (kRouteMaxDepth - 2);
struct RouteArgs {
  GrowState gs; TreeArrays tree; const uint8_t* bins_col; int64_t n;
  uint8_t* node_of_row;
  unsigned* tile_counts;
  unsigned ntiles; int has_missing, level;
  const float* g; const float2* gpair; int g_only; const unsigned* tail_row;
  unsigned* ridx; void* gp; unsigned* tl;
  unsigned long long* rows_counter;
};

struct HistArgs {
  const uint8_t* bins;
  const uint8_t* bins_tail;
  const unsigned* tail_pos;
  int64_t n;
  int row_stride;
  const uint8_t* bins_gather;
  int gather_stride;
  int tail_in_gather;
  int tw;
  const float2* gpair;
  const float* gpos;
  const unsigned* ridx;
  const int* build_count;
  const int* build_nid;
  const unsigned* build_prefix;
  const unsigned* seg_begin;
  const int* hist_slot;
  const float* scales;
  GH64* hist_pool;
  GH64* node_sum;
  int ngroups;
  int ng_chunk;
  int accumulate_sum;
  int g_only;
  int window_rows;
  int force_gather;
  unsigned long long* rows_counter;
};

constexpr int kLgRootSlot = 0, kLgStageSlot = 1, kLgFirstFreeSlot = 2;
void launch_apply_lossguide(const ApplyArgs& a, int iter, cudaStream_t s);
void launch_lg_copy_back(const PartArgs& a, unsigned* ridx_dst, void* gp_dst, unsigned* tl_dst, unsigned max_tiles, cudaStream_t s);
void launch_zero_build_slots(const GrowState& gs, GH64* pool, size_t slot_entries, int max_build, cudaStream_t s);
void launch_lg_stage(const GrowState& gs, GH64* pool, size_t slot_entries, int to_stage, cudaStream_t s);
void launch_hist_build(const HistArgs& a, int num_sms, cudaStream_t stream);
void hist_configure();
const char* hist_last_kernel();
void launch_init_tree(const GrowState& gs, const TreeArrays& t, unsigned n, cudaStream_t s);
void launch_scales(const GrowState& gs, int grad_bits, cudaStream_t s);
void launch_eval(const EvalArgs& a, int max_nodes_level, cudaStream_t s);
void launch_apply(const ApplyArgs& a, cudaStream_t s);
void launch_partition(const PartArgs& a, unsigned max_tiles, cudaStream_t s);
void launch_route(const RouteArgs& a, cudaStream_t s);
void launch_update_margin(const TreeArrays& t, const int* n_nodes, const uint8_t* bins_col, int64_t n, int has_missing, const uint8_t* node_of_row,
                          float* margin, int K, int k, const float* leaf_scale, cudaStream_t s);
void launch_subtract(const GrowState& gs, GH64* pool, size_t slot_entries, int max_build, cudaStream_t s);

}
```

Measured before the change: 102.3.

## Use thread-block clusters for deep histogram gather with DSMEM reduction flush

```diff
diff --git a/microbench/deep_hist_profile.py b/microbench/deep_hist_profile.py
--- /dev/null
+++ b/microbench/deep_hist_profile.py
@@ -0,0 +1,87 @@
+#!/usr/bin/env python
+import argparse
+import json
+import os
+import sys
+
+ROOT = os.path.dirname(os.path.dirname(os.path.abspath(__file__)))
+sys.path.insert(0, ROOT)
+
+GATHER_ROW_BYTES = 140
+
+
+def main():
+    ap = argparse.ArgumentParser()
+    ap.add_argument("--rows", type=int, default=50_000_000)
+    ap.add_argument("--cols", type=int, default=100)
+    ap.add_argument("--max-depth", type=int, default=6)
+    ap.add_argument("--objective", default="reg:squarederror")
+    ap.add_argument("--warmup", type=int, default=5)
+    ap.add_argument("--timed", type=int, default=10)
+    ap.add_argument("--profiled", type=int, default=3)
+    ap.add_argument("--out", default="")
+    a = ap.parse_args()
+    import torch
+    import bench
+    import sagemaker_xgboost_container_b200 as xgb
+    be = xgb.get_backend()
+    dev = torch.device("cuda", 0)
+    ba = argparse.Namespace(rows=a.rows, cols=a.cols, seed=43, objective=a.objective, num_class=0)
+    X, y = bench.gen_shard(ba, 0, a.rows, dev)
+    d = xgb.DMatrix(X, label=y.cpu().numpy())
+    del X
+    torch.cuda.empty_cache()
+    params = bench.params_of(argparse.Namespace(objective=a.objective, max_depth=a.max_depth, max_bin=256, num_class=0))
+    b = xgb.Booster(params, [d])
+    it = 0
+    for _ in range(a.warmup):
+        b.update(d, it); it += 1
+    be.synchronize()
+    be.timer_start()
+    for _ in range(a.timed):
+        b.update(d, it); it += 1
+    round_ms = be.timer_stop() / a.timed
+    be.booster_set_profile(b.handle, True)
+    for _ in range(a.profiled):
+        b.update(d, it); it += 1
+    p = be.booster_get_profile(b.handle)
+    be.booster_set_profile(b.handle, False)
+    R = a.profiled
+    levels = []
+    tot = {"ms": 0.0, "flush_ms": 0.0, "segments": 0.0}
+    for lvl, c in enumerate(p["hist_level_counters"]):
+        cyc = {k: c[k + "_cycles"] for k in ("zero", "stream", "switch", "final")}
+        total = sum(cyc.values())
+        share = {k: (v / total if total else 0.0) for k, v in cyc.items()}
+        ms = p["deep_hist_level_ms"][lvl - 1] / R if lvl >= 1 else None
+        rows = c["rows"] / R
+        e = {"level": lvl, "rows": rows, "segments": c["segments"] / R, "ctas": c["ctas"] / R, "cluster": c["cluster"], "cycle_share": share}
+        if ms is not None:
+            e["ms"] = ms
+            e["gbs_at_140B"] = rows * GATHER_ROW_BYTES / (ms * 1e-3) / 1e9 if ms > 0 else 0.0
+            e["flush_ms"] = ms * (share["switch"] + share["final"])
+            tot["ms"] += ms; tot["flush_ms"] += e["flush_ms"]; tot["segments"] += e["segments"]
+        levels.append(e)
+    name = torch.cuda.get_device_name(dev)
+    try:
+        import pynvml
+        pynvml.nvmlInit()
+        power_w = pynvml.nvmlDeviceGetPowerManagementLimit(pynvml.nvmlDeviceGetHandleByIndex(0)) / 1000.0
+    except Exception:
+        power_w = None
+    out = {"gpu": name, "power_limit_w": power_w, "rows": a.rows, "cols": a.cols, "objective": a.objective, "max_depth": a.max_depth,
+           "profiled_rounds": R, "round_ms": round_ms, "root_hist_ms": p["root_hist_ms"] / R,
+           "deep_hist_ms": p["deep_hist_ms"] / R, "deep_levels": tot, "levels": levels, "profile": p}
+    for e in levels:
+        s = e["cycle_share"]
+        when = "%.3f ms (%.0f GB/s at 140 B/row, flush ~%.3f ms)" % (e["ms"], e["gbs_at_140B"], e["flush_ms"]) if "ms" in e else "root pass"
+        print("level %d: %s, rows %.1fM, segments %.0f, CTAs %.0f (cluster %d); cycles: zero %.3f stream %.3f switch %.3f final %.3f" % (
+            e["level"], when, e["rows"] / 1e6, e["segments"], e["ctas"], e["cluster"], s["zero"], s["stream"], s["switch"], s["final"]),
+            flush=True)
+    print(json.dumps(out), flush=True)
+    if a.out:
+        json.dump(out, open(a.out, "w"), indent=1)
+
+
+if __name__ == "__main__":
+    main()
diff --git a/sagemaker-xgboost-container_b200/csrc/grow.cu b/sagemaker-xgboost-container_b200/csrc/grow.cu
--- a/sagemaker-xgboost-container_b200/csrc/grow.cu
+++ b/sagemaker-xgboost-container_b200/csrc/grow.cu
@@ -174,9 +174,9 @@
   if (in.n_ic > 0) { aa.node_path = ic_path.p; aa.node_allowed = ic_allowed.p; aa.ic_sets = ic_sets.p; aa.n_ic_sets = in.n_ic; aa.F = bm.F; }
   return aa;
 }
-template <class Launch> void TreeBuilder::timed(ProfKind kind, Launch launch) {
+template <class Launch> void TreeBuilder::timed(ProfKind kind, Launch launch, int level) {
   if (!profile) { launch(); return; }
-  ProfEvent e; e.kind = kind; e.launches = g_kernel_launches;
+  ProfEvent e; e.kind = kind; e.launches = g_kernel_launches; e.level = level;
   CUDA_OK(cudaEventCreate(&e.a)); CUDA_OK(cudaEventCreate(&e.b));
   CUDA_OK(cudaEventRecord(e.a, engine_stream()));
   launch();
@@ -210,7 +210,7 @@
   }
   HistArgs root = hist_args(bm, k);
   if (g_only) { root.gpair = nullptr; root.gpos = g_dense(); }
-  root.g_only = in.root_mode == 2 ? 1 : 0; root.rows_counter = profile ? prof_rows.p : nullptr;
+  root.g_only = in.root_mode == 2 ? 1 : 0; root.rows_counter = profile ? prof_rows.p : nullptr; root.prof = profile ? prof_hist.p : nullptr;
   timed(kProfRootHist, [&] { launch_hist_build(root, num_sms, s); });
   if (in.root_mode == 1) { snapshot_h_kernel<<<num_sms, 256, 0, s>>>(hist_pool.p, root_h_cache.p, slot_stride); ++g_kernel_launches; CUDA_OK(cudaGetLastError()); }
   auto collective = [&](std::function<void()> f) {
@@ -240,11 +240,11 @@
     pa.has_missing = bm.has_missing; pa.level = level; pa.max_level_nodes = max_level_nodes; pa.rows_counter = profile ? prof_rows.p + 2 : nullptr;
     return pa;
   };
-  auto level_hist_args = [&](int set) {
+  auto level_hist_args = [&](int set, int level) {
     HistArgs ha = hist_args(bm, k);
     ha.ridx = ridx[set].p; ha.tail_pos = carry_tail ? tl[set].p : nullptr; ha.accumulate_sum = 0;
     ha.gpair = g_only ? nullptr : gp[set].p; ha.gpos = g_only ? reinterpret_cast<const float*>(gp[set].p) : nullptr;
-    ha.rows_counter = profile ? prof_rows.p + 1 : nullptr;
+    ha.rows_counter = profile ? prof_rows.p + 1 : nullptr; ha.prof = profile ? prof_hist.p + (size_t)level * kHistProfN : nullptr;
     return ha;
   };
   launch_eval(eval_args(in, 0, in.mask), 1, s);
@@ -254,7 +254,7 @@
     timed(kProfPartition, [&] { launch_partition(pa, max_tiles, s); });
     launch_lg_copy_back(pa, ridx[0].p, gp[0].p, tl[0].p, max_tiles, s);
     launch_zero_build_slots(gs, hist_pool.p, slot_stride, 1, s);
-    timed(kProfDeepHist, [&] { launch_hist_build(level_hist_args(0), num_sms, s); });
+    timed(kProfDeepHist, [&] { launch_hist_build(level_hist_args(0, 1), num_sms, s); }, 1);
     if (dist) {
       launch_lg_stage(gs, hist_pool.p, slot_stride, 1, s);
       allreduce_hist(hist_pool.p + (size_t)kLgStageSlot * slot_stride, slot_stride * 2);
@@ -282,7 +282,7 @@
       timed(kProfPartition, [&] { launch_partition(pa, max_tiles, s); });
     }
     CUDA_OK(cudaMemsetAsync(hist_pool.p + (size_t)next_base * slot_stride, 0, (size_t)next_half * slot_stride * sizeof(GH64), s));
-    timed(kProfDeepHist, [&] { launch_hist_build(level_hist_args(routed ? 0 : L & 1), num_sms, s); });
+    timed(kProfDeepHist, [&] { launch_hist_build(level_hist_args(routed ? 0 : L & 1, L + 1), num_sms, s); }, L + 1);
     allreduce_hist(hist_pool.p + (size_t)next_base * slot_stride, (size_t)next_half * slot_stride * 2);
     launch_subtract(gs, hist_pool.p, slot_stride, next_half, s);
     launch_eval(eval_args(in, L + 1, in.mask ? in.mask + (size_t)(L + 1) * bm.F : nullptr), 1 << (L + 1), s);
@@ -451,7 +451,10 @@
 
 void TreeBuilder::set_profile(bool on) {
   profile = on;
-  if (on) { prof_rows.alloc(4); prof_rows.zero(engine_stream()); prof_margin_rows = 0; }
+  if (on) {
+    prof_rows.alloc(4); prof_rows.zero(engine_stream()); prof_margin_rows = 0;
+    prof_hist.alloc((size_t)(kMaxDepth + 1) * kHistProfN); prof_hist.zero(engine_stream());
+  }
   for (auto& e : prof_events) { cudaEventDestroy(e.a); cudaEventDestroy(e.b); }
   prof_events.clear();
 }
@@ -469,7 +472,27 @@
            ms[kProfRootHist], launches[kProfRootHist], rows[0], ms[kProfDeepHist], launches[kProfDeepHist], rows[1],
            ms[kProfPartition], launches[kProfPartition], rows[2], rows[3], prof_part_row_bytes[0], prof_part_row_bytes[1], prof_part_row_bytes[2],
            ms[kProfMargin], launches[kProfMargin], prof_margin_rows);
-  return buf;
-}
-
-}
+  double level_ms[kMaxDepth + 1] = {};
+  int deepest = 0;
+  for (auto& e : prof_events)
+    if (e.kind == kProfDeepHist && e.level > 0) { float t = 0; CUDA_OK(cudaEventElapsedTime(&t, e.a, e.b)); level_ms[e.level] += t; deepest = std::max(deepest, e.level); }
+  std::vector<unsigned long long> hp((size_t)(kMaxDepth + 1) * kHistProfN, 0);
+  if (prof_hist.p) CUDA_OK(cudaMemcpy(hp.data(), prof_hist.p, hp.size() * sizeof(unsigned long long), cudaMemcpyDeviceToHost));
+  std::string o(buf);
+  o.pop_back();
+  o += ",\"deep_hist_level_ms\":[";
+  for (int l = 1; l <= deepest; ++l) { snprintf(buf, sizeof buf, "%s%.6f", l > 1 ? "," : "", level_ms[l]); o += buf; }
+  o += "],\"deep_hist_level_rows\":[";
+  for (int l = 1; l <= deepest; ++l) o += (l > 1 ? "," : "") + std::to_string(hp[(size_t)l * kHistProfN + kHistProfRows]);
+  o += "],\"hist_level_counters\":[";
+  const char* names[kHistProfN] = {"zero_cycles", "stream_cycles", "switch_cycles", "final_cycles", "segments", "ctas", "rows", "cluster"};
+  for (int l = 0; l <= deepest; ++l) {
+    o += l ? ",{" : "{";
+    for (int i = 0; i < kHistProfN; ++i) o += std::string(i ? "," : "") + "\"" + names[i] + "\":" + std::to_string(hp[(size_t)l * kHistProfN + i]);
+    o += "}";
+  }
+  o += "]}";
+  return o;
+}
+
+}
diff --git a/sagemaker-xgboost-container_b200/csrc/grow.h b/sagemaker-xgboost-container_b200/csrc/grow.h
--- a/sagemaker-xgboost-container_b200/csrc/grow.h
+++ b/sagemaker-xgboost-container_b200/csrc/grow.h
@@ -82,8 +82,9 @@
   int max_leaves() const { return lg_iters > 0 ? lg_iters + 1 : 1 << max_depth; }
   float* ensure_adaptive();
   enum ProfKind { kProfRootHist, kProfDeepHist, kProfPartition, kProfMargin, kProfKinds };
-  struct ProfEvent { cudaEvent_t a, b; int kind; long long launches; };
+  struct ProfEvent { cudaEvent_t a, b; int kind; long long launches; int level; };
   bool profile = false; std::vector<ProfEvent> prof_events;
+  DevBuf<unsigned long long> prof_hist;
   DevBuf<unsigned long long> prof_rows;
   long long prof_margin_rows = 0;
   int prof_part_row_bytes[3] = {0, 0, 0};
@@ -111,7 +112,7 @@
   float* g_dense() const { return reinterpret_cast<float*>(gpair.p); }
   EvalArgs eval_args(const TreeInputs& in, int level, const unsigned char* feat_mask) const;
   ApplyArgs apply_args(const TreeInputs& in, int level, int next_base, int next_half) const;
-  template <class Launch> void timed(ProfKind kind, Launch launch);
+  template <class Launch> void timed(ProfKind kind, Launch launch, int level = -1);
 };
 
 }
diff --git a/sagemaker-xgboost-container_b200/csrc/hist.cu b/sagemaker-xgboost-container_b200/csrc/hist.cu
--- a/sagemaker-xgboost-container_b200/csrc/hist.cu
+++ b/sagemaker-xgboost-container_b200/csrc/hist.cu
@@ -12,9 +12,14 @@
 
 constexpr int kSuperRows = 32;
 constexpr int kMinRowsPerCta = 4096;
-constexpr int kSpillThreshold = 1 << 24;
+constexpr int kSpillThresholdG = 1 << 25;
+constexpr unsigned kSpillThresholdH = 1u << 26;
+static_assert((long long)(kSpillThresholdG - 1) + (long long)kWindowRows * (1LL << kGradBits) < (1LL << 31) &&
+              (long long)(kSpillThresholdG - 1) + (long long)kWindowRowsSmall * (1LL << kGradBitsSmall) < (1LL << 31), "G plane overflow");
+static_assert((long long)(kSpillThresholdH - 1) + (long long)kWindowRows * (1LL << (kGradBits + 1)) < (1LL << 32) &&
+              (long long)(kSpillThresholdH - 1) + (long long)kWindowRowsSmall * (1LL << (kGradBitsSmall + 1)) < (1LL << 32), "H plane overflow");
 constexpr int kPlaneBytes = kGroupEntries * 4;
-constexpr int kMaxSmem = 232448;
+constexpr int kMaxSmem = 232448 - 128;
 constexpr int kTeamWarps = 4, kTeams = 6, kRootRows = 16 * kTeamWarps;
 constexpr int kRootConsumerWarps = kTeamWarps * kTeams;
 constexpr int kRootProducerWarps = 3;
@@ -108,6 +113,18 @@
 __device__ __forceinline__ void named_bar_sync(int id, int nthreads) {
   asm volatile("bar.sync %0, %1;" :: "r"(id), "r"(nthreads) : "memory");
 }
+__device__ __forceinline__ unsigned cluster_nctarank() { unsigned r; asm("mov.u32 %0, %%cluster_nctarank;" : "=r"(r)); return r; }
+__device__ __forceinline__ void cluster_barrier() {
+  asm volatile("barrier.cluster.arrive.release.aligned;\n\tbarrier.cluster.wait.acquire.aligned;" ::: "memory");
+}
+__device__ __forceinline__ unsigned map_shared_rank(unsigned addr, unsigned rank) {
+  unsigned r; asm volatile("mapa.shared::cluster.u32 %0, %1, %2;" : "=r"(r) : "r"(addr), "r"(rank)); return r;
+}
+__device__ __forceinline__ int4 ld_cluster_v4(unsigned addr) {
+  int4 r;
+  asm volatile("ld.shared::cluster.v4.s32 {%0,%1,%2,%3}, [%4];" : "=r"(r.x), "=r"(r.y), "=r"(r.z), "=r"(r.w) : "r"(addr) : "memory");
+  return r;
+}
 
 struct LaneConst { unsigned A[16]; unsigned S[4]; int qw; };
 
@@ -198,6 +215,20 @@
     red_shared_s32(addr, gq);
     red_shared_u32(addr + kHPlane, hq);
   }
+}
+
+struct HistProf { long long mark, cyc[4], segs; };
+__device__ __forceinline__ void prof_start(HistProf& p) {
+  p.mark = clock64(); p.segs = 0;
+#pragma unroll
+  for (int i = 0; i < 4; ++i) p.cyc[i] = 0;
+}
+__device__ __forceinline__ void prof_charge(HistProf& p, int phase) { const long long t = clock64(); p.cyc[phase] += t - p.mark; p.mark = t; }
+__device__ __forceinline__ void prof_commit(const HistProf& p, unsigned long long* dst) {
+#pragma unroll
+  for (int i = 0; i < 4; ++i) atomicAdd(dst + i, (unsigned long long)p.cyc[i]);
+  atomicAdd(dst + kHistProfSegments, (unsigned long long)p.segs);
+  atomicAdd(dst + kHistProfCtas, 1ull);
 }
 
 __device__ __forceinline__ void flush_node_sum(GH64* dst, int g, unsigned h, int lane) {
@@ -224,7 +255,7 @@
 #pragma unroll
     for (int k = 0; k < 4; ++k) {
       const int val = vals[k];
-      const bool sp = last ? (val != 0) : (is_h ? ((unsigned)val >= (unsigned)kSpillThreshold) : (val >= kSpillThreshold || val <= -kSpillThreshold));
+      const bool sp = last ? (val != 0) : (is_h ? ((unsigned)val >= kSpillThresholdH) : (val >= kSpillThresholdG || val <= -kSpillThresholdG));
       if (sp) {
         red_global_s64(is_h ? &o[k].h : &o[k].g, is_h ? (long long)(unsigned)val : (long long)val);
         vals[k] = 0; any = true;
@@ -244,11 +275,45 @@
     const bool is_h = idx >= per_plane;
     const int e = is_h ? idx - per_plane : idx;
     const int bin = e / per_bin, slot = e & (tw - 1);
-    const bool sp = last ? true : (is_h ? ((unsigned)val >= (unsigned)kSpillThreshold) : (val >= kSpillThreshold || val <= -kSpillThreshold));
+    const bool sp = last ? true : (is_h ? ((unsigned)val >= kSpillThresholdH) : (val >= kSpillThresholdG || val <= -kSpillThresholdG));
     if (sp) {
       GH64* o = out_tail + bin * tw + slot;
       red_global_s64(is_h ? &o->h : &o->g, is_h ? (long long)(unsigned)val : (long long)val);
       tsm[idx] = 0;
+    }
+  }
+}
+
+template <int NG, int TWC, int TREP>
+__device__ __forceinline__ void flush_cluster(unsigned smem_addr, int ng_here, bool has_tail, GH64* out_main, GH64* out_tail, unsigned K,
+                                              unsigned rank, unsigned cl, unsigned ncl, int tid, int nthr) {
+  constexpr int kTailVec = NG * 2 * (kGroupEntries / 4);
+  constexpr int kTailPlane = 256 * TWC * TREP;
+  const int vmain = ng_here * 2 * (kGroupEntries / 4);
+  const int V = vmain + (has_tail ? 2 * kTailPlane / 4 : 0);
+  const int lo = (int)((long long)V * rank / K), len = (int)((long long)V * (rank + 1) / K) - lo;
+  const int start = (int)((long long)cl * len / ncl);
+  for (int i = tid; i < len; i += nthr) {
+    int j = i + start; if (j >= len) j -= len;
+    const int v = lo + j;
+    const bool main = v < vmain;
+    const unsigned addr = smem_addr + 16u * (unsigned)(main ? v : kTailVec + (v - vmain));
+    const int t0 = (v - vmain) * 4;
+    const bool is_h = main ? ((v >> 11) & 1) != 0 : t0 >= kTailPlane;
+    long long s[4] = {0, 0, 0, 0};
+    for (unsigned r = 0; r < K; ++r) {
+      const int4 x = ld_cluster_v4(r == rank ? addr : map_shared_rank(addr, r));
+      if (is_h) { s[0] += (unsigned)x.x; s[1] += (unsigned)x.y; s[2] += (unsigned)x.z; s[3] += (unsigned)x.w; }
+      else { s[0] += x.x; s[1] += x.y; s[2] += x.z; s[3] += x.w; }
+    }
+    if ((s[0] | s[1] | s[2] | s[3]) == 0) continue;
+#pragma unroll
+    for (int k = 0; k < 4; ++k) {
+      if (s[k] == 0) continue;
+      GH64* o;
+      if (main) o = out_main + (size_t)(v >> 12) * kGroupEntries + ((v & 2047) << 2) + k;
+      else { const int e = (is_h ? t0 - kTailPlane : t0) + k; o = out_tail + (e / (TWC * TREP)) * TWC + (e & (TWC - 1)); }
+      red_global_s64(is_h ? &o->h : &o->g, s[k]);
     }
   }
 }
@@ -288,6 +353,11 @@
   const int ng_here = min(a.ng_chunk, a.ngroups - g0);
   const bool has_tail = a.tw > 0 && blockIdx.y == gridDim.y - 1;
   if (a.rows_counter && blockIdx.x == 0 && blockIdx.y == 0 && threadIdx.x == 0) atomicAdd(a.rows_counter, (unsigned long long)T);
+  __shared__ HistProf prof;
+  if (a.prof && threadIdx.x == 0) {
+    prof_start(prof);
+    if (blockIdx.x == 0 && blockIdx.y == 0) atomicAdd(a.prof + kHistProfRows, (unsigned long long)T);
+  }
 
   const unsigned smem_base = (unsigned)__cvta_generic_to_shared(smem_raw);
   const unsigned ring = (smem_base + c.ring_off + 127u) & ~127u;
@@ -314,6 +384,7 @@
     }
   }
   __syncthreads();
+  if (a.prof && threadIdx.x == 0) prof_charge(prof, kHistProfZero);
 
   const int nid = a.build_nid[0];
   const size_t slot_entries = (size_t)a.ngroups * kGroupEntries + (size_t)256 * a.tw;
@@ -411,6 +482,7 @@
     if (has_tail) spill_tail<PL>(reinterpret_cast<int*>(smem_raw + c.tail_off), a.tw, c.trep, out_tail, false, threadIdx.x, NCW * 32);
     named_bar_sync(1, NCW * 32);
   }
+  if (a.prof && threadIdx.x == 0) prof_charge(prof, kHistProfStream);
   named_bar_sync(1, NCW * 32);
   spill_main<PL>(reinterpret_cast<int*>(smem_raw), ng_here, out_main, true, threadIdx.x, NCW * 32);
   if (has_tail) spill_tail<PL>(reinterpret_cast<int*>(smem_raw + c.tail_off), a.tw, c.trep, out_tail, true, threadIdx.x, NCW * 32);
@@ -419,6 +491,7 @@
     for (int o = 16; o > 0; o >>= 1) { accG += __shfl_xor_sync(0xffffffffu, accG, o); accH += __shfl_xor_sync(0xffffffffu, accH, o); }
     if (lane == 0 && (accG != 0 || accH != 0)) { red_global_s64(&a.node_sum[nid].g, accG); red_global_s64(&a.node_sum[nid].h, accH); }
   }
+  if (a.prof && threadIdx.x == 0) { prof_charge(prof, kHistProfFinal); prof.segs = 1; prof_commit(prof, a.prof); }
 }
 
 template <int TW, bool GPAY> struct Stage { unsigned id; typename std::conditional<GPAY, float, float2>::type gr; unsigned t0; };
@@ -441,14 +514,19 @@
   const unsigned T = a.build_prefix[nb];
   if (T == 0) return;
   if (a.rows_counter && blockIdx.x == 0 && blockIdx.y == 0 && threadIdx.x == 0) atomicAdd(a.rows_counter, (unsigned long long)T);
-  const unsigned C = gridDim.x;
-  unsigned ceff = (T + kMinRowsPerCta - 1) / kMinRowsPerCta;
+  const unsigned K = cluster_nctarank(), C = gridDim.x / K, cl = blockIdx.x / K;
+  unsigned ceff = (T + K * kMinRowsPerCta - 1) / (K * kMinRowsPerCta);
   ceff = ceff < 1 ? 1 : (ceff > C ? C : ceff);
-  if (blockIdx.x >= ceff) return;
+  if (cl >= ceff) return;
   unsigned chunk = (T + ceff - 1) / ceff;
-  chunk = (chunk + SUP - 1) / SUP * SUP;
-  unsigned long long r0l = (unsigned long long)blockIdx.x * chunk;
+  chunk = (chunk + K * SUP - 1) / (K * SUP) * (K * SUP);
+  unsigned long long r0l = (unsigned long long)cl * chunk;
   if (r0l >= T) return;
+  __shared__ HistProf prof;
+  if (a.prof && threadIdx.x == 0) {
+    prof_start(prof);
+    if (blockIdx.x == 0 && blockIdx.y == 0) { atomicAdd(a.prof + kHistProfRows, (unsigned long long)T); atomicMax(a.prof + kHistProfCluster, (unsigned long long)K); }
+  }
   unsigned r0 = (unsigned)r0l;
   unsigned r1 = (unsigned long long)r0 + chunk > T ? T : r0 + chunk;
   const int g0 = blockIdx.y * a.ng_chunk;
@@ -476,6 +554,7 @@
     for (int i = threadIdx.x; i < words4; i += NTHREADS) reinterpret_cast<int4*>(smem)[i] = make_int4(0, 0, 0, 0);
   }
   __syncthreads();
+  if (a.prof && threadIdx.x == 0) prof_charge(prof, kHistProfZero);
 
   int b = 0;
   { int lo = 0, hi = nb; while (lo < hi) { int mid = (lo + hi) >> 1; if (a.build_prefix[mid + 1] > r0) hi = mid; else lo = mid + 1; } b = lo; }
@@ -494,7 +573,8 @@
     int accG = 0; unsigned accH = 0;
     const unsigned pa = seg + (r0 - nbeg), pb = seg + (nend - nbeg);
     const unsigned nsuper = (pb - pa + SUP - 1) / SUP;
-    const unsigned iters = (nsuper + NWARPS - 1) / NWARPS;
+    const unsigned iters = (nsuper + K * NWARPS - 1) / (K * NWARPS);
+    const unsigned s0 = blockIdx.x % K + K * warp;
 
     auto load_ids = [&](unsigned st) -> StageT {
       StageT s_; s_.id = 0xffffffffu; s_.gr = {}; s_.t0 = 0u;
@@ -523,15 +603,15 @@
         }
       }
     };
-    StageT cur = load_ids(warp);
-    StageT nxt = load_ids(warp + NWARPS);
+    StageT cur = load_ids(s0);
+    StageT nxt = load_ids(s0 + K * NWARPS);
     uint4 w[U];
 #pragma unroll
     for (int k = 0; k < U; ++k) w[k] = load_unit(cur.id, k);
     load_line_tail(cur);
     for (unsigned it = 0; it < iters; ++it) {
-      const unsigned s = warp + it * NWARPS;
-      StageT nn = load_ids(s + 2 * NWARPS);
+      const unsigned s = s0 + it * (K * NWARPS);
+      StageT nn = load_ids(s + 2 * K * NWARPS);
       const bool active = s < nsuper;
       int gq_l; unsigned hq_l;
       if constexpr (GPAY) { gq_l = __float2int_rn(cur.gr * sg); hq_l = cur.id != 0xffffffffu ? hq_one : 0u; }
@@ -560,13 +640,27 @@
         __syncthreads();
       }
     }
-    __syncthreads();
-    spill_main<2>(smem, ng_here, out_main, true, threadIdx.x, NTHREADS);
-    if (has_tail) spill_tail<2>(smem + NG * 2 * kGroupEntries, TWC, trep, out_tail, true, threadIdx.x, NTHREADS);
-    __syncthreads();
+    if (a.prof && threadIdx.x == 0) prof_charge(prof, kHistProfStream);
     if (a.accumulate_sum && blockIdx.y == 0) flush_node_sum(a.node_sum + nid, accG, accH, lane);
     r0 = nend; ++b;
-  }
+    if (K > 1) {
+      cluster_barrier();
+      flush_cluster<NG, TWC, trep>(smem_g, ng_here, has_tail, out_main, out_tail, K, blockIdx.x % K, cl, ceff, threadIdx.x, NTHREADS);
+      cluster_barrier();
+      if (r0 < r1) {
+        const int words4 = (NG * 2 * kPlaneBytes + (TAIL ? 2 * 256 * TWC * trep * 4 : 0)) / 16;
+        for (int i = threadIdx.x; i < words4; i += NTHREADS) reinterpret_cast<int4*>(smem)[i] = make_int4(0, 0, 0, 0);
+        __syncthreads();
+      }
+    } else {
+      __syncthreads();
+      spill_main<2>(smem, ng_here, out_main, true, threadIdx.x, NTHREADS);
+      if (has_tail) spill_tail<2>(smem + NG * 2 * kGroupEntries, TWC, trep, out_tail, true, threadIdx.x, NTHREADS);
+      __syncthreads();
+    }
+    if (a.prof && threadIdx.x == 0) { prof_charge(prof, r0 < r1 ? kHistProfSwitch : kHistProfFinal); ++prof.segs; }
+  }
+  if (a.prof && threadIdx.x == 0) prof_commit(prof, a.prof);
 }
 
 static thread_local const char* g_last_kernel = "none";
@@ -631,29 +725,65 @@
   return true;
 }
 
-template <int NG, int TW, int NT> static void set_gather_attr() {
-  const int smem = NG * 2 * kPlaneBytes + (TW ? gather_tail_bytes(NG) : 0);
-  CUDA_OK(cudaFuncSetAttribute(hist_gather_kernel<NG, TW, NT, false>, cudaFuncAttributeMaxDynamicSharedMemorySize, smem));
-  CUDA_OK(cudaFuncSetAttribute(hist_gather_kernel<NG, TW, NT, true>, cudaFuncAttributeMaxDynamicSharedMemorySize, smem));
+struct GatherPlan { int K = 1, clusters = 0; };
+template <int NG, int TW, int NT, bool GPAY> static GatherPlan& gather_plan() { static GatherPlan p; return p; }
+template <int NG, int TW, int NT> constexpr int gather_smem() { return NG * 2 * kPlaneBytes + (TW ? gather_tail_bytes(NG) : 0); }
+
+template <int NG, int TW, int NT, bool GPAY> static void plan_gather(bool clusters) {
+  auto kern = hist_gather_kernel<NG, TW, NT, GPAY>;
+  constexpr int smem = gather_smem<NG, TW, NT>();
+  CUDA_OK(cudaFuncSetAttribute(kern, cudaFuncAttributeMaxDynamicSharedMemorySize, smem));
+  GatherPlan& p = gather_plan<NG, TW, NT, GPAY>();
+  p = GatherPlan{};
+  if (!clusters) return;
+  int dev = 0, nsm = 0, per_sm = 0;
+  CUDA_OK(cudaGetDevice(&dev));
+  CUDA_OK(cudaDeviceGetAttribute(&nsm, cudaDevAttrMultiProcessorCount, dev));
+  CUDA_OK(cudaOccupancyMaxActiveBlocksPerMultiprocessor(&per_sm, kern, NT, smem));
+  for (int K : {4, 2}) {
+    cudaLaunchConfig_t cfg = {};
+    cfg.gridDim = dim3(K); cfg.blockDim = dim3(NT); cfg.dynamicSmemBytes = smem;
+    cudaLaunchAttribute at; at.id = cudaLaunchAttributeClusterDimension; at.val.clusterDim.x = K; at.val.clusterDim.y = 1; at.val.clusterDim.z = 1;
+    cfg.attrs = &at; cfg.numAttrs = 1;
+    int n = 0;
+    if (cudaOccupancyMaxActiveClusters(&n, kern, &cfg) != cudaSuccess) { cudaGetLastError(); n = 0; }
+    if (n > 0 && n * K >= nsm * per_sm) { p.K = K; p.clusters = n; return; }
+  }
+}
+template <int NG, int TW, int NT> static void plan_gather_both(bool clusters) {
+  plan_gather<NG, TW, NT, false>(clusters); plan_gather<NG, TW, NT, true>(clusters);
 }
 
 void hist_configure() {
   static bool configured = false;
   if (configured) return;
-  set_gather_attr<1, 0, 256>(); set_gather_attr<1, 4, 256>(); set_gather_attr<1, 8, 256>();
-  set_gather_attr<2, 0, 768>(); set_gather_attr<2, 4, 768>(); set_gather_attr<2, 8, 768>();
-  set_gather_attr<3, 0, 768>(); set_gather_attr<3, 4, 768>(); set_gather_attr<3, 8, 768>();
+  const bool cl = getenv("B200XGB_NO_CLUSTER_HIST") == nullptr || strcmp(getenv("B200XGB_NO_CLUSTER_HIST"), "0") == 0;
+  plan_gather_both<1, 0, 256>(cl); plan_gather_both<1, 4, 256>(cl); plan_gather_both<1, 8, 256>(cl);
+  plan_gather_both<2, 0, 768>(cl); plan_gather_both<2, 4, 768>(cl); plan_gather_both<2, 8, 768>(cl);
+  plan_gather_both<3, 0, 768>(cl); plan_gather_both<3, 4, 768>(cl); plan_gather_both<3, 8, 768>(cl);
   CUDA_OK(cudaFuncSetAttribute(hist_root_kernel<false>, cudaFuncAttributeMaxDynamicSharedMemorySize, kMaxSmem));
   CUDA_OK(cudaFuncSetAttribute(hist_root_kernel<true>, cudaFuncAttributeMaxDynamicSharedMemorySize, kMaxSmem));
   configured = true;
 }
 
+template <int NG, int TW, int NT, bool GPAY>
+static void launch_gather_kernel(const HistArgs& a, int gx, int nchunks, cudaStream_t stream) {
+  const GatherPlan& p = gather_plan<NG, TW, NT, GPAY>();
+  cudaLaunchConfig_t cfg = {};
+  cfg.gridDim = dim3(gx, nchunks); cfg.blockDim = dim3(NT); cfg.dynamicSmemBytes = gather_smem<NG, TW, NT>(); cfg.stream = stream;
+  cudaLaunchAttribute at;
+  if (p.K > 1 && p.clusters / nchunks > 0) {
+    cfg.gridDim.x = (unsigned)(p.clusters / nchunks * p.K);
+    at.id = cudaLaunchAttributeClusterDimension; at.val.clusterDim.x = p.K; at.val.clusterDim.y = 1; at.val.clusterDim.z = 1;
+    cfg.attrs = &at; cfg.numAttrs = 1;
+  }
+  CUDA_OK(cudaLaunchKernelEx(&cfg, hist_gather_kernel<NG, TW, NT, GPAY>, a));
+}
 template <int NG, int NT, bool GPAY>
 static void launch_gather_tw(const HistArgs& a, int gx, int nchunks, cudaStream_t stream) {
-  const int smem = NG * 2 * kPlaneBytes + (a.tw ? gather_tail_bytes(NG) : 0);
-  if (a.tw == 0) hist_gather_kernel<NG, 0, NT, GPAY><<<dim3(gx, nchunks), NT, smem, stream>>>(a);
-  else if (a.tw == 4) hist_gather_kernel<NG, 4, NT, GPAY><<<dim3(gx, nchunks), NT, smem, stream>>>(a);
-  else hist_gather_kernel<NG, 8, NT, GPAY><<<dim3(gx, nchunks), NT, smem, stream>>>(a);
+  if (a.tw == 0) launch_gather_kernel<NG, 0, NT, GPAY>(a, gx, nchunks, stream);
+  else if (a.tw == 4) launch_gather_kernel<NG, 4, NT, GPAY>(a, gx, nchunks, stream);
+  else launch_gather_kernel<NG, 8, NT, GPAY>(a, gx, nchunks, stream);
 }
 template <int NG, int NT>
 static void launch_gather(const HistArgs& a, int gx, int nchunks, cudaStream_t stream) {
diff --git a/sagemaker-xgboost-container_b200/csrc/tree.h b/sagemaker-xgboost-container_b200/csrc/tree.h
--- a/sagemaker-xgboost-container_b200/csrc/tree.h
+++ b/sagemaker-xgboost-container_b200/csrc/tree.h
@@ -76,7 +76,9 @@
   int window_rows;
   int force_gather;
   unsigned long long* rows_counter;
+  unsigned long long* prof;
 };
+enum { kHistProfZero, kHistProfStream, kHistProfSwitch, kHistProfFinal, kHistProfSegments, kHistProfCtas, kHistProfRows, kHistProfCluster, kHistProfN };
 
 constexpr int kLgRootSlot = 0, kLgStageSlot = 1, kLgFirstFreeSlot = 2;
 void launch_apply_lossguide(const ApplyArgs& a, int iter, cudaStream_t s);
```

Result: faster. 105.1 (median of 6 runs) (+2.7%).
